# pandegroup/deepchem

Measured on AMD Instinct MI355X. Metric: molecules/sec fwd+bwd GraphConvModel, higher is better.
Workload: dtype f32; 1 GPU; Tox21-like synthetic molecules (18.2 atoms/mol, E/N 2.08), 12 binary tasks, GraphConvModel [64,64]/dense 128, BatchNorm on, fwd+bwd+Adam per step; grad_mode=full, gemm_mode=fast (split-bf16 x3 products on v_mfma_f32_32x32x16_bf16, fp32-accurate), parallelism=dp1 (molecules sharded by rank, one flat all-reduce per step)

## Files before the change

### deepchem_amd/_lib.py

```python
import ctypes
import os
from ctypes import (POINTER, Structure, c_char_p, c_double, c_float, c_int32, c_int64, c_void_p)

from deepchem_amd import _build

GCMI_MAX_DEG = 10
BN_ACC_REPLICAS = 32


def bn_acc_doubles(n_feat: int) -> int:
    return 66 * n_feat
K_GATHER_SUM, K_GATHER_MAX, K_READOUT, K_SEG_GEMM, K_WGRAD, K_GATHER_MAX_BWD, K_BATCHNORM, K_FUSED_BWD = 0, 1, 2, 3, 4, 5, 6, 7


GCMI_OPT_GEMM_EXACT = 1
GCMI_OPT_FUSED_BN_STATS = 2
GCMI_OPT_FUSED_BWD = 3
GCMI_OPT_FUSED_BWD_LAUNCHES = 4
GCMI_OPT_READOUT_PIPELINED = 5
GCMI_OPT_ONE_PIECE_LAUNCHES = 6
GCMI_OPT_MAX_SUM_LAUNCHES = 7
GCMI_METRIC_ROC_AUC, GCMI_METRIC_PRC_AUC = 0, 1
GCMI_METRIC_MOMENTS, GCMI_METRIC_ACCURACY = 0, 1
GCMI_METRIC_MOMENT_DOUBLES = 12
GCMI_WIN_META_INTS = 24
GCMI_COLLATE_WIN_DESC_INTS = 36
GCMI_WIN_MAX_SLOTS = 4095


class GcmiGraph(Structure):
    _fields_ = [
        ("n_atoms", c_int32),
        ("n_edges", c_int32),
        ("n_mols", c_int32),
        ("max_deg", c_int32),
        ("deg_start", c_int32 * (GCMI_MAX_DEG + 2)),
        ("edge_start", c_int32 * (GCMI_MAX_DEG + 2)),
        ("d_col_idx", c_void_p),
        ("d_membership", c_void_p),
        ("d_mol_runs", c_void_p),
        ("d_rev_pos", c_void_p),
        ("n_win", c_int32),
        ("n_win_big", c_int32),
        ("win_alloc", c_int32),
        ("win_ecap", c_int32),
        ("win_alloc_big", c_int32),
        ("win_ecap_big", c_int32),
        ("win_reserved", c_int32 * 2),
        ("d_win_meta", c_void_p),
        ("d_win_edges", c_void_p),
    ]


MAX_CONV_LAYERS = 4


class GcmiModelDesc(Structure):
    _fields_ = [
        ("n_layers", c_int32),
        ("max_deg", c_int32),
        ("n_feat_in", c_int32),
        ("conv_width", c_int32 * MAX_CONV_LAYERS),
        ("dense_width", c_int32),
        ("n_tasks", c_int32),
        ("n_classes", c_int32),
        ("mode", c_int32),
        ("batch_norm", c_int32),
        ("grad_mode", c_int32),
        ("bn_eps", c_float),
        ("bn_momentum", c_float),
        ("off_conv_w", c_int64 * MAX_CONV_LAYERS),
        ("off_conv_b", c_int64 * MAX_CONV_LAYERS),
        ("off_bn_gamma", c_int64 * (MAX_CONV_LAYERS + 1)),
        ("off_bn_beta", c_int64 * (MAX_CONV_LAYERS + 1)),
# ... 260 lines not shown
```

### deepchem_amd/csrc/bn.hip

```cpp
#include "common.h"
#include "split_bf16.h"

namespace gcmi {

constexpr int kBBlock = 256;
constexpr int kRowsPerBlock = 512;
constexpr int kResidentBlocks = 2048;
constexpr int kReplicas = kBnReplicas;

template <int V>
__device__ __forceinline__ void readout_dy(const ReadoutGrad& rg, int64_t r, int c, int n_feat, float (&dy)[V]) {
  const int m = rg.membership[r];
  const float* grow = rg.g2 + (int64_t)m * rg.ldg2;
  const int32_t* arow = rg.arg + (int64_t)m * n_feat;
  if constexpr (V == 4) {
    const float4 s4 = *reinterpret_cast<const float4*>(grow + c);
    const float4 m4 = *reinterpret_cast<const float4*>(grow + n_feat + c);
    const int4 a4 = *reinterpret_cast<const int4*>(arow + c);
    dy[0] = s4.x + (a4.x == r ? m4.x : 0.f);
    dy[1] = s4.y + (a4.y == r ? m4.y : 0.f);
    dy[2] = s4.z + (a4.z == r ? m4.z : 0.f);
    dy[3] = s4.w + (a4.w == r ? m4.w : 0.f);
  } else {
    dy[0] = grow[c] + (arow[c] == r ? grow[n_feat + c] : 0.f);
// ... 322 lines not shown
    const int c = cc * V;
    float A[V], B[V], C[V];
#pragma unroll
    for (int q = 0; q < V; ++q) {
      A[q] = coef[c + q];
      B[q] = coef[n_feat + c + q];
      C[q] = coef[2 * n_feat + c + q];
    }
    constexpr int R = 4;
    for (int64_t r0 = r_begin + ty; r0 < r_end; r0 += (int64_t)R * ry) {
      float xv[R][V], gv[R][V];
#pragma unroll
      for (int u = 0; u < R; ++u) {
        const int64_t r = r0 + (int64_t)u * ry;
        const int64_t rc = r < r_end ? r : r_end - 1;
        if constexpr (RD) readout_dy<V>(rg, rc, c, n_feat, gv[u]);
        if constexpr (V == 4) {
          const float4 a4 = *reinterpret_cast<const float4*>(x + rc * ldx + c);
          xv[u][0] = a4.x; xv[u][1] = a4.y; xv[u][2] = a4.z; xv[u][3] = a4.w;
          if (!RD) {
            const float4 b4 = *reinterpret_cast<const float4*>(dy + rc * lddy + c);
            gv[u][0] = b4.x; gv[u][1] = b4.y; gv[u][2] = b4.z; gv[u][3] = b4.w;
          }
        } else {
          xv[u][0] = x[rc * ldx + c];
          if (!RD) gv[u][0] = dy[rc * lddy + c];
        }
      }
#pragma unroll
      for (int u = 0; u < R; ++u) {
        const int64_t r = r0 + (int64_t)u * ry;
        if (r >= r_end) continue;
        float o[V];
#pragma unroll
        for (int q = 0; q < V; ++q) {
          const float v = fmaf(A[q], gv[u][q], fmaf(B[q], xv[u][q], C[q]));
          o[q] = (RELU && !(xv[u][q] > 0.f)) ? 0.f : v;
        }
        if constexpr (V == 4) {
          *reinterpret_cast<float4*>(dx + r * lddx + c) = make_float4(o[0], o[1], o[2], o[3]);
        } else {
          dx[r * lddx + c] = o[0];
        }
      }
    }
  }
}

static int launch_col_sums(int mode, const float* a, int64_t lda, const float* x, int64_t ldx,
                           const float* mean, const float* invstd, int64_t n_rows, int n_feat,
                           double* sums, bool acc_clean, hipStream_t st, const ReadoutGrad* rgp = nullptr,
                           const float* only_if_gamma = nullptr, const float* only_if_beta = nullptr, int x_bf16 = 0) {
  if (!acc_clean &&
      hipMemsetAsync(sums, 0, sizeof(double) * 2 * n_feat * (1 + kReplicas), st) != hipSuccess) {
    set_error("bn: memset failed");
    return GCMI_ERR_LAUNCH;
  }
  if (n_rows == 0) return GCMI_OK;
  ReadoutGrad rg{nullptr, nullptr, 0, nullptr};
  int V;
  if (rgp) {
    rg = *rgp;
    mode = 2;
    V = (vec_width(x, ldx, n_feat) == 4 && aligned16(rg.g2) && rg.ldg2 % 4 == 0 && aligned16(rg.arg)) ? 4 : 1;
  } else if (x_bf16) {
    const bool a_ok = x_bf16 == 2 ? ((reinterpret_cast<uintptr_t>(a) & 7u) == 0 && lda % 4 == 0 && n_feat % 4 == 0)
                                  : vec_width(a, lda, n_feat) == 4;
    if (mode != 1 || !a_ok || (reinterpret_cast<uintptr_t>(x) & 7u) || ldx % 4) {
      set_error("bn col_sums: bf16 rows need mode 1 and 8-byte addressable rows");
      return GCMI_ERR_UNSUPPORTED;
    }
    V = 4;
  } else {
    V = vec_width(a, lda, n_feat);
    if (mode == 1 && vec_width(x, ldx, n_feat) != 4) V = 1;
  }
  const int lpr = n_feat / V;
  const int lx = lpr < kBBlock ? lpr : kBBlock;
  const int64_t round_rows = 4 * (kBBlock / lx);
  int64_t rpb = (n_rows + kResidentBlocks - 1) / kResidentBlocks;
  if (rpb < kRowsPerBlock) rpb = kRowsPerBlock;
  rpb = (rpb + round_rows - 1) / round_rows * round_rows;
  const int blocks = (int)((n_rows + rpb - 1) / rpb);
  const int rev = next_sweep_direction();
#define LAUNCH_CS(VV, MM)                                                                     \
  hipLaunchKernelGGL((col_sums_kernel<VV, MM>), dim3(blocks), dim3(kBBlock), 0, st, a, lda, x, \
                     ldx, mean, invstd, n_rows, rpb, n_feat, lpr, lx, sums, rg, rev, only_if_gamma, only_if_beta)
  if (x_bf16 == 2) {
    hipLaunchKernelGGL((col_sums_kernel<4, 1, true, true>), dim3(blocks), dim3(kBBlock), 0, st, a, lda, x, ldx, mean, invstd,
                       n_rows, rpb, n_feat, lpr, lx, sums, rg, rev, only_if_gamma, only_if_beta);
  } else if (x_bf16) {
    hipLaunchKernelGGL((col_sums_kernel<4, 1, true>), dim3(blocks), dim3(kBBlock), 0, st, a, lda, x, ldx, mean, invstd,
                       n_rows, rpb, n_feat, lpr, lx, sums, rg, rev, only_if_gamma, only_if_beta);
  } else if (V == 4) {
    if (mode == 0) LAUNCH_CS(4, 0); else if (mode == 1) LAUNCH_CS(4, 1); else LAUNCH_CS(4, 2);
  } else {
    if (mode == 0) LAUNCH_CS(1, 0); else if (mode == 1) LAUNCH_CS(1, 1); else LAUNCH_CS(1, 2);
  }
#undef LAUNCH_CS
  GCMI_CHECK_LAUNCH("bn col_sums");
  return GCMI_OK;
}

static int bn_sync_collapse(const BnPoint& p, int64_t n_rows, double* d_acc, double* d_psums, double* d_xbuf, hipStream_t st,
                            const BnBackward::Loss& loss = {}) {
  static_assert(kReplicas == 32, "bn_collapse_kernel: one lane per replica");
  hipLaunchKernelGGL(bn_collapse_kernel, dim3((p.n_feat + 7) / 8), dim3(256), 0, st, d_acc, d_psums, n_rows, p.n_feat, p.gamma,
                     p.beta, p.dgamma, p.dbeta, d_xbuf, loss.acc, loss.rep, loss.inv_count, loss.out);
  GCMI_CHECK_LAUNCH("bn_collapse");
  return GCMI_OK;
}

static int bn_sync_exchange(const BnSync& sy, int64_t n_rows, int32_t n_feat, hipStream_t st) {
  const int64_t n = 2 * (int64_t)n_feat + 1;
  if (n_rows == 0 && hipMemsetAsync(sy.buf, 0, sizeof(double) * (size_t)n, st) != hipSuccess) {
    set_error("bn sync: memset failed");
    return GCMI_ERR_LAUNCH;
  }
  if (sy.fn(sy.ctx, sy.buf, n, st) != 0) {
    set_error("synchronised BatchNorm: the statistics exchange callback failed");
    return GCMI_ERR_LAUNCH;
  }
  return GCMI_OK;
}

static int bn_sync_finalize(const BnPoint& p, const double* d_xbuf, hipStream_t st) {
  hipLaunchKernelGGL(bn_finalize_sync_kernel, dim3((p.n_feat + 255) / 256), dim3(256), 0, st, d_xbuf, p.n_feat, p.gamma,
                     p.beta, p.eps, p.momentum, p.running_mean, p.running_var, p.mean, p.invstd, p.scale, p.shift,
                     p.batches_tracked);
  GCMI_CHECK_LAUNCH("bn_finalize_sync");
  return GCMI_OK;
}

int bn_train_forward(const BnPoint& p, const BnForward& f, void* stream) {
  const int32_t n_feat = p.n_feat;
  if (f.sync) {
    GCMI_CHECK_ARG(n_feat > 0 && f.n_rows >= 0 && p.scale && p.shift && f.acc && f.sync->fn && f.sync->buf,
                   "bn_stats_sync: bad arguments");
    GCMI_CHECK_ARG(f.n_rows == 0 || f.sums_ready || (f.x && f.ldx >= n_feat), "bn_stats_sync: bad rows");
  } else if (f.sums_ready) {
    GCMI_CHECK_ARG(n_feat > 0 && f.n_rows > 0 && p.scale && p.shift && f.acc, "bn_finalize: bad arguments");
  } else {
    GCMI_CHECK_ARG(n_feat > 0 && f.n_rows > 0 && f.ldx >= n_feat, "bn_stats: bad shape (n_rows=%lld)", (long long)f.n_rows);
    GCMI_CHECK_ARG(f.x && p.scale && p.shift && f.acc, "bn_stats: NULL buffer");
  }
  hipStream_t st = (hipStream_t)stream;
  TimedScope ts(GCMI_K_BATCHNORM, st);
  int rc = GCMI_OK;
  if (f.n_rows > 0 && !f.sums_ready)
    rc = launch_col_sums(0, f.x, f.ldx, nullptr, 0, nullptr, nullptr, f.n_rows, n_feat, f.acc, f.acc_clean, st);
  if (rc) return rc;
  if (!f.sync) {
    hipLaunchKernelGGL(bn_finalize_kernel, dim3((n_feat + 7) / 8), dim3(256), 0, st, f.acc, f.n_rows, n_feat, p.gamma, p.beta,
                       p.eps, p.momentum, p.running_mean, p.running_var, p.mean, p.invstd, p.scale, p.shift, p.batches_tracked);
    GCMI_CHECK_LAUNCH("bn_finalize");
    return GCMI_OK;
  }
  if (f.n_rows > 0) rc = bn_sync_collapse(BnPoint{n_feat}, f.n_rows, f.acc, nullptr, f.sync->buf, st);
  if (rc == GCMI_OK) rc = bn_sync_exchange(*f.sync, f.n_rows, n_feat, st);
  if (rc) return rc;
  return bn_sync_finalize(p, f.sync->buf, st);
}

static int bn_bwd_sync_finish(const BnPoint& p, const BnBackward& b, hipStream_t st) {
  const BnSync& sy = *b.sync;
  GCMI_CHECK_ARG(p.n_feat > 0 && b.n_rows > 0 && sy.fn && sy.buf, "bn_bwd_sync: bad arguments");
  GCMI_CHECK_ARG(p.mean && p.invstd && b.acc, "bn_bwd_sync: NULL buffer");
  int rc = bn_sync_collapse(p, b.n_rows, b.acc, b.psums, sy.buf, st, b.loss);
// ... 217 lines not shown
}

int bn_bwd_pool_impl(const BnPoint& p, const BnBackward& b, void* stream) {
  const int32_t n_feat = p.n_feat;
  GCMI_CHECK_ARG(n_feat > 0 && b.n_rows > 0 && p.mean && p.invstd && b.acc && b.psums && b.x && p.gamma && p.beta,
                 "bn_bwd_pool: bad arguments");
  hipStream_t st = (hipStream_t)stream;
  TimedScope ts(GCMI_K_BATCHNORM, st);
  if (b.dy != nullptr) {
    const int rc = launch_col_sums(1, b.dy, b.lddy, b.x, b.ldx, p.mean, p.invstd, b.n_rows, n_feat, b.acc, true, st, nullptr,
                                   p.gamma, p.beta, b.x_bf16);
    if (rc) return rc;
  }
  if (b.sync != nullptr) return bn_bwd_sync_finish(p, b, st);
  static_assert(kReplicas == 32, "bn_bwd_params_pool_kernel: one lane per replica");
  hipLaunchKernelGGL(bn_bwd_params_pool_kernel, dim3((n_feat + 7) / 8), dim3(256), 0, st, b.psums, b.acc, b.n_rows, n_feat,
                     p.gamma, p.beta, p.mean, p.invstd, p.dgamma, p.dbeta, reinterpret_cast<float*>(b.acc));
  GCMI_CHECK_LAUNCH("bn_bwd_params_pool");
  return GCMI_OK;
}

static int bn_bwd_params(const BnPoint& p, const BnBackward& b, hipStream_t st) {
  hipLaunchKernelGGL(bn_bwd_params_kernel, dim3((p.n_feat + 7) / 8), dim3(256), 0, st, b.acc, b.n_rows, p.n_feat, p.gamma,
                     p.mean, p.invstd, p.dgamma, p.dbeta, reinterpret_cast<float*>(b.acc), b.loss.acc, b.loss.rep,
                     b.loss.inv_count, b.loss.out);
  GCMI_CHECK_LAUNCH("bn_bwd_params");
  return GCMI_OK;
}

int bn_bwd_params_impl(const BnPoint& p, const BnBackward& b, void* stream) {
  GCMI_CHECK_ARG(p.n_feat > 0 && b.n_rows > 0 && p.mean && p.invstd && b.acc, "bn_bwd_params: bad arguments");
  hipStream_t st = (hipStream_t)stream;
  TimedScope ts(GCMI_K_BATCHNORM, st);
  return b.sync != nullptr ? bn_bwd_sync_finish(p, b, st) : bn_bwd_params(p, b, st);
}

int bn_bwd_impl(const BnPoint& p, const BnBackward& b, void* stream) {
  const int32_t n_feat = p.n_feat;
  const int64_t n_rows = b.n_rows;
  const ReadoutGrad* rgp = b.rg;
  if (rgp)
    GCMI_CHECK_ARG(rgp->membership && rgp->g2 && rgp->arg && rgp->ldg2 >= 2 * (int64_t)n_feat,
                   "bn_bwd_readout: bad readout gradient");
  else
    GCMI_CHECK_ARG(b.lddy >= n_feat && b.dy, "bn_bwd: bad dy");
  GCMI_CHECK_ARG(n_feat > 0 && n_rows > 0 && b.ldx >= n_feat, "bn_bwd: bad shape");
  GCMI_CHECK_ARG(b.x && p.mean && p.invstd && b.acc, "bn_bwd: NULL buffer");
  GCMI_CHECK_ARG(b.dx == nullptr || b.lddx >= n_feat, "bn_bwd: bad lddx");
  hipStream_t st = (hipStream_t)stream;
  TimedScope ts(GCMI_K_BATCHNORM, st);
  int rc = GCMI_OK;
  if (rgp && rgp->rawsum && rgp->runs && rgp->n_mols > 0) {
    if (!b.acc_clean &&
        hipMemsetAsync(b.acc, 0, sizeof(double) * 2 * n_feat * (1 + kReplicas), st) != hipSuccess) {
      set_error("bn: memset failed");
      return GCMI_ERR_LAUNCH;
    }
    const int chunks = (n_feat + 63) / 64;
    int waves = 4096 / chunks * chunks;
    const int64_t jobs = (int64_t)rgp->n_mols * chunks;
    if (jobs < waves) waves = (int)((jobs + chunks - 1) / chunks * chunks);
    const int blocks = (waves + 3) / 4;
    hipLaunchKernelGGL(readout_bn_sums_kernel, dim3(blocks), dim3(256), 0, st, rgp->n_mols, n_feat, rgp->n_deg,
                       rgp->runs, rgp->g2, rgp->ldg2, rgp->arg, rgp->rawsum, b.x, b.ldx, p.mean, p.invstd, chunks,
                       b.acc);
    GCMI_CHECK_LAUNCH("readout_bn_sums");
  } else {
    rc = launch_col_sums(1, b.dy, b.lddy, b.x, b.ldx, p.mean, p.invstd, n_rows, n_feat, b.acc, b.acc_clean, st, rgp);
  }
  if (rc) return rc;
  rc = b.sync != nullptr ? bn_bwd_sync_finish(p, b, st) : bn_bwd_params(p, b, st);
  if (rc) return rc;
  if (b.dx) {
    const float* coef = reinterpret_cast<const float*>(b.acc);
    ReadoutGrad rg{nullptr, nullptr, 0, nullptr};
    if (rgp) rg = *rgp;
    const bool src_ok = rgp ? (aligned16(rg.g2) && rg.ldg2 % 4 == 0 && aligned16(rg.arg))
                            : vec_width(b.dy, b.lddy, n_feat) == 4;
    const int V = (vec_width(b.dx, b.lddx, n_feat) == 4 && src_ok && vec_width(b.x, b.ldx, n_feat) == 4) ? 4 : 1;
    const int lpr = n_feat / V;
    const int lx = lpr < kBBlock ? lpr : kBBlock;
    const int64_t round_rows = 4 * (kBBlock / lx);
    int64_t rpb = (n_rows + kResidentBlocks - 1) / kResidentBlocks;
    if (rpb < kDxRows) rpb = kDxRows;
    rpb = (rpb + round_rows - 1) / round_rows * round_rows;
    const int blocks = (int)((n_rows + rpb - 1) / rpb);
    const int rev = next_sweep_direction();
#define LAUNCH_DX(VV, RR, DD)                                                                     \
  hipLaunchKernelGGL((bn_bwd_dx_kernel<VV, RR, DD>), dim3(blocks), dim3(kBBlock), 0, st, b.dy, b.lddy, \
                     b.x, b.ldx, n_rows, rpb, n_feat, lpr, lx, coef, b.dx, b.lddx, rg, rev)
#define LAUNCH_DX_R(VV, RR) \
  do { if (rgp) LAUNCH_DX(VV, RR, true); else LAUNCH_DX(VV, RR, false); } while (0)
    if (V == 4) {
      if (b.relu_mask) LAUNCH_DX_R(4, true); else LAUNCH_DX_R(4, false);
    } else {
      if (b.relu_mask) LAUNCH_DX_R(1, true); else LAUNCH_DX_R(1, false);
    }
#undef LAUNCH_DX_R
#undef LAUNCH_DX
    GCMI_CHECK_LAUNCH("bn_bwd_dx");
  }
  return GCMI_OK;
}

}
```

### deepchem_amd/csrc/bwd_fused.hip

```cpp
#include <atomic>
#include <type_traits>

#include "common.h"
#include "split_bf16.h"

namespace gcmi {

constexpr int kFRows = 64;

struct FusedArgs {
  const float* dy;
  int32_t lddy;
  const float* x;
  int32_t ldx;
  const float* coef;
  const int32_t* membership;
  const float* g2;
  int32_t ldg2;
  const int32_t* arg;
  const float* in[2];
  int32_t ldin[2];
  int32_t k_in;
  const float* w;
  float* dw;
// ... 519 lines not shown
    if (stamp) { t0 = wall_clock64(); d_w2 += t0 - t1; }
    prow0 = row0; pvalid = valid; pseg = seg;
    seg = nseg; row0 = nrow0; valid = nvalid;
    nseg = n2seg; nrow0 = n2row0; nvalid = n2valid;
  }
  store_out(prow0, pvalid, pseg);
  if (!is_dgrad) flush_w(cur_seg);
  if constexpr (DGRAD) {
    if (a.psums != nullptr) {
      flush_psums();
      __syncthreads();
      for (int c = tid; c < 2 * KP; c += NT) {
        const int which = c / KP, col = c - which * KP;
        if (col < a.k_in)
          atomicAdd(a.psums + (size_t)2 * a.k_in * (1 + (blockIdx.x % kBnReplicas)) + (size_t)which * a.k_in + col,
                    stat_s[which][col]);
      }
    }
  }
  if (stamp) {
    unsigned long long* d = a.diag + (wave == 0 ? 0 : 5);
    d[0] = d_a; d[1] = d_w1; d[2] = d_b; d[3] = d_w2; d[4] = (unsigned long long)my_tiles;
  }
}

static bool fused_bwd_on() {
  static const int env = getenv("GCMI_FUSED_BWD") ? atoi(getenv("GCMI_FUSED_BWD")) : 1;
  return env != 0;
}

static std::atomic<int> g_fused_bwd{1};
static std::atomic<int> g_fused_launches{0};
int fused_bwd_launches() { return g_fused_launches.load(std::memory_order_relaxed); }
void set_fused_bwd(int on) { g_fused_bwd.store(on ? 1 : 0, std::memory_order_relaxed); }
int get_fused_bwd() { return g_fused_bwd.load(std::memory_order_relaxed); }
bool fused_bwd_enabled() { return fused_bwd_on() && get_fused_bwd() != 0 && !gemm_exact_mode(); }

template <int NG, int KT, int NOPS, bool TRANS, bool RD, bool DGRAD, bool HB = false, bool GB = false, bool IB = HB>
static int launch_fused(const SegTable& st, int n_tiles, const FusedArgs& a, hipStream_t sm) {
  constexpr int KP = KT * 32;
  size_t shmem = sizeof(float) * kFRows * (NG + 4) + sizeof(float) * (size_t)NOPS * kFRows * (KP + 4);
  if (DGRAD)
    shmem += sizeof(unsigned short) * (size_t)NOPS * 3 * KP * (NG + 8) + sizeof(float) * kFRows * (NOPS * KT * 32 + 8);
  auto kern = fused_bwd_kernel<NG, KT, NOPS, TRANS, RD, DGRAD, HB, GB, IB>;
  static LdsLimit lim;
  if (!raise_lds_limit(lim, reinterpret_cast<const void*>(kern), shmem)) return GCMI_ERR_UNSUPPORTED;
  const int per_cu = DGRAD ? 1 : 2;
  const int grid = std::min(n_tiles, 256 * per_cu);
  static const bool diag_on = getenv("GCMI_FUSED_DIAG") && atoi(getenv("GCMI_FUSED_DIAG")) != 0;
  static unsigned long long* d_diag = nullptr;
  FusedArgs aa = a;
  if (diag_on) {
    if (!d_diag && hipMalloc(&d_diag, 10 * sizeof(unsigned long long)) != hipSuccess) d_diag = nullptr;
    if (d_diag) (void)hipMemsetAsync(d_diag, 0, 10 * sizeof(unsigned long long), sm);
    aa.diag = d_diag;
  }
  hipLaunchKernelGGL(kern, dim3(grid), dim3(DGRAD ? 512 : 256), shmem, sm, st, n_tiles, aa, next_sweep_direction());
  GCMI_CHECK_LAUNCH("fused_bwd");
  if (diag_on && d_diag) {
    unsigned long long h[10];
    if (hipStreamSynchronize(sm) == hipSuccess && hipMemcpy(h, d_diag, sizeof(h), hipMemcpyDeviceToHost) == hipSuccess)
      fprintf(stderr, "fused_bwd<%d,%d,%d> tiles %llu | first wave: G phase %.2f us, wait %.2f, products %.2f, wait %.2f "
                      "| last wave: %.2f %.2f %.2f %.2f (per tile)\n", NG, KT, (int)DGRAD, h[4],
              h[0] * 0.01 / h[4], h[1] * 0.01 / h[4], h[2] * 0.01 / h[4], h[3] * 0.01 / h[4], h[5] * 0.01 / h[4],
              h[6] * 0.01 / h[4], h[7] * 0.01 / h[4], h[8] * 0.01 / h[4]);
  }
  g_fused_launches.fetch_add(1, std::memory_order_relaxed);
  return GCMI_OK;
}

static FusedArgs fused_args(const BlockBackward& b) {
  FusedArgs a;
  memset(&a, 0, sizeof(a));
  a.dy = b.dy; a.lddy = (int32_t)b.lddy; a.x = b.gc; a.ldx = (int32_t)b.ldgc; a.coef = b.coef;
  if (b.rg) { a.membership = b.rg->membership; a.g2 = b.rg->g2; a.ldg2 = (int32_t)b.rg->ldg2; a.arg = b.rg->arg; }
  for (int o = 0; o < 2; ++o) {
    a.in[o] = b.in[o].rows; a.ldin[o] = (int32_t)b.in[o].ld;
    a.dout[o] = b.dout[o].rows; a.lddout[o] = (int32_t)b.dout[o].ld;
  }
  a.k_in = b.k_in; a.w = b.w; a.dw = b.dw; a.db = b.db;
  a.psums = b.dout[0].rows ? b.psums : nullptr;
  return a;
}

int fused_conv_bwd(const BlockBackward& b, hipStream_t sm) {
  const int32_t k_in = b.k_in, act_bf16 = b.act_bf16, in_bf16 = b.in_bf16;
  if (!fused_bwd_enabled() || b.n_seg > kMaxProductSeg || b.width != 64 || b.rg != nullptr) return GCMI_ERR_UNSUPPORTED;
  if (in_bf16 && (act_bf16 || b.dout[0].rows != nullptr || k_in <= 64 || k_in > 96)) return GCMI_ERR_UNSUPPORTED;
  {
    int64_t rows = 0;
    for (int sgi = 0; sgi < b.n_seg; ++sgi) rows = std::max<int64_t>(rows, b.seg_end[sgi]);
    const int64_t ldmax = std::max(std::max(b.lddy, b.ldgc),
                                   std::max(std::max(b.in[0].ld, b.in[1].ld), std::max(b.dout[0].ld, b.dout[1].ld)));
    if (rows * ldmax >= (int64_t)1 << 30) return GCMI_ERR_UNSUPPORTED;
  }
  if (!aligned16(b.dy) || b.lddy % 4 || !aligned16(b.gc) || b.ldgc % 4) return GCMI_ERR_UNSUPPORTED;
  if (b.coef && !aligned16(b.coef)) return GCMI_ERR_UNSUPPORTED;
  if ((act_bf16 || in_bf16) && (!aligned16(b.in[0].rows) || b.in[0].ld % 4 || !aligned16(b.in[1].rows) || b.in[1].ld % 4))
    return GCMI_ERR_UNSUPPORTED;
  const bool dgrad = b.dout[0].rows != nullptr;
  SegTable st;
  const int tiles = (int)fill_seg_table(st, b.n_seg, b.seg_begin, b.seg_end, b.w_off[0], b.w_off[1], b.b_off, kFRows);
  if (tiles == 0) return GCMI_OK;
  const FusedArgs a = fused_args(b);
  if (dgrad) {
    if (k_in % 4 || b.dout[0].ld % 4 || b.dout[1].ld % 4 || !aligned16(b.dout[0].rows) || !aligned16(b.dout[1].rows))
      return GCMI_ERR_UNSUPPORTED;
// ... 124 lines not shown
```

### deepchem_amd/csrc/collate.cpp

```cpp
#include <cmath>
#include <algorithm>
#include <cstdlib>
#include <string>
#include <thread>
#include <vector>

#include "common.h"

namespace {

constexpr int ND = GCMI_MAX_DEG + 1;

template <typename F>
void parallel_for(int64_t n, int n_threads, F&& fn) {
  if (n_threads <= 1 || n < 512) {
    fn(0, n, 0);
    return;
  }
  std::vector<std::thread> th;
  for (int t = 0; t < n_threads; ++t) th.emplace_back(fn, n * t / n_threads, n * (t + 1) / n_threads, t);
  for (auto& x : th) x.join();
}


// ... 686 lines not shown
    for (int d = 0; d < ND; ++d) {
      D[d] = W.begin[d];
      D[ND + d] = W.sb[d];
      D[2 * ND + d] = W.eb[d];
    }
    GCMI_CHECK_ARG(W.eoff < (1LL << 31), "collate: window entries exceed int32");
    D[3 * ND] = (int32_t)W.eoff;
    D[3 * ND + 1] = D[3 * ND + 2] = 0;
  }
  out_offsets[0] = o_base;
  out_offsets[1] = o_win;
  out_offsets[2] = o_off;
  out_offsets[3] = o_a0;
  out_offsets[4] = o_meta;
  out_offsets[5] = o_desc;
  out_offsets[6] = o_desc + n_win * WD;
  out_offsets[7] = P.want_win ? P.win_entries : 0;
  graph->n_atoms = (int32_t)P.n_atoms;
  graph->n_edges = (int32_t)P.n_edges;
  graph->n_mols = (int32_t)n_sel;
  graph->max_deg = max_deg;
  for (int d = 0; d < GCMI_MAX_DEG + 2; ++d) {
    graph->deg_start[d] = (int32_t)P.deg_start[d <= n_deg ? d : n_deg];
    graph->edge_start[d] = (int32_t)P.edge_start[d <= n_deg ? d : n_deg];
  }
  graph->d_col_idx = nullptr;
  graph->d_membership = nullptr;
  graph->d_mol_runs = nullptr;
  graph->d_rev_pos = nullptr;
  graph->n_win = (int32_t)n_win;
  graph->n_win_big = P.want_win ? P.n_win_big : 0;
  graph->win_alloc = P.want_win ? P.win_alloc : 0;
  graph->win_ecap = P.want_win ? P.win_ecap : 0;
  graph->win_alloc_big = P.want_win ? P.win_alloc_big : 0;
  graph->win_ecap_big = P.want_win ? P.win_ecap_big : 0;
  graph->win_reserved[0] = P.want_win ? P.n_mols_with_atoms : 0;
  graph->win_reserved[1] = 0;
  graph->d_win_meta = nullptr;
  graph->d_win_edges = nullptr;
  return GCMI_OK;
}

int gcmi_collate_rows(const void* d_features, int64_t n_feat, const int64_t* d_adj_ptr, const int32_t* d_adj_idx,
                      const int32_t* d_rank, const uint8_t* d_rev, const int32_t* d_staging, const int64_t* offsets,
                      const gcmi_graph* plan, float* d_out_features, int64_t out_ld, int32_t* d_membership,
                      int32_t* d_col_idx, int32_t* d_mol_runs, uint8_t* d_rev_pos, uint16_t* d_win_edges,
                      int64_t* d_src_atom, void* stream_) {
  hipStream_t stream = (hipStream_t)stream_;
  RowsArgs A;
  const int rc = fill_rows_args(A, d_features, n_feat, d_adj_ptr, d_adj_idx, d_rank, d_rev, d_staging, offsets, plan,
                                d_out_features, out_ld, d_membership, d_col_idx, d_mol_runs, d_rev_pos, d_win_edges);
  if (rc != GCMI_OK) return rc;
  if (A.want_win && offsets[7] > 0)
    if (hipMemsetAsync(d_win_edges, 0, (size_t)offsets[7] * sizeof(uint16_t), stream) != hipSuccess) {
      ::gcmi::set_error("collate_rows: hipMemsetAsync failed");
      return GCMI_ERR_LAUNCH;
    }
  A.src_atom = d_src_atom;
  if (A.n_atoms > 0) {
    collate_rows_kernel<<<(unsigned)((A.n_atoms + 255) / 256), 256, 0, stream>>>(A);
    GCMI_CHECK_LAUNCH("collate_rows_kernel");
    if (d_src_atom) {
      const int64_t n_el = (int64_t)A.n_atoms * A.out_ld;
      GCMI_CHECK_ARG(n_el / 256 < (1LL << 31), "collate_rows: feature block too large for one launch");
      if (A.out_ld % 4 == 0 && ((uintptr_t)A.out_feat & 15) == 0 && n_el / 4 < (1LL << 31)) {
        const uint32_t n_quads = (uint32_t)(n_el / 4);
        collate_features_quad_kernel<<<(n_quads + 255u) / 256u, 256, 0, stream>>>(A, (uint32_t)(A.out_ld / 4), n_quads);
      } else {
        collate_features_kernel<<<(unsigned)((n_el + 255) / 256), 256, 0, stream>>>(A);
      }
      GCMI_CHECK_LAUNCH("collate_features_kernel");
    }
  }
  const int64_t n_runs = (int64_t)A.n_sel * A.n_deg;
  if (d_mol_runs && n_runs > 0) {
    collate_runs_kernel<<<(unsigned)((n_runs + 255) / 256), 256, 0, stream>>>(A);
    GCMI_CHECK_LAUNCH("collate_runs_kernel");
  }
  return GCMI_OK;
}

int gcmi_collate_rows_host(const void* features, int64_t n_feat, const int64_t* adj_ptr, const int32_t* adj_idx,
                           const int32_t* rank, const uint8_t* rev, const int32_t* staging, const int64_t* offsets,
                           const gcmi_graph* plan, float* out_features, int64_t out_ld, int32_t* membership,
                           int32_t* col_idx, int32_t* mol_runs, uint8_t* rev_pos, uint16_t* win_edges) {
  RowsArgs A;
  const int rc = fill_rows_args(A, features, n_feat, adj_ptr, adj_idx, rank, rev, staging, offsets, plan, out_features,
                                out_ld, membership, col_idx, mol_runs, rev_pos, win_edges);
  if (rc != GCMI_OK) return rc;
  if (A.want_win)
    for (int64_t q = 0; q < offsets[7]; ++q) win_edges[q] = 0;
  for (int32_t i = 0; i < A.n_atoms; ++i) collate_atom(A, i);
  if (mol_runs)
    for (int64_t k = 0; k < (int64_t)A.n_sel * A.n_deg; ++k) collate_run(A, (int32_t)k);
  return GCMI_OK;
}

}

namespace {
inline int64_t up4w(int64_t n) { return (n + 3) / 4 * 4; }
}

extern "C" {

int64_t gcmi_collate_batches_layout(const int64_t* atom_ptr, const int64_t* adj_ptr, const int64_t* sel,
                                    const int64_t* batch_ptr, int64_t n_batches, int64_t ld, int32_t max_deg,
// ... 127 lines not shown
```

### deepchem_amd/csrc/common.h

```cpp
#pragma once
#include <hip/hip_runtime.h>
#include <algorithm>
#include <atomic>
#include <stdlib.h>
#include <stdint.h>
#include <stdio.h>
#include <string.h>

#include "../../include/gcmi.h"

namespace gcmi {

void set_error(const char* fmt, ...);
int next_sweep_direction();

constexpr int kMaxDev = 64;
struct LdsLimit {
  std::atomic<int> per_cu[kMaxDev];
};
int raise_lds_limit(LdsLimit& a, const void* kern, size_t lds_bytes, int threads = 0, size_t shmem = 0);

#define GCMI_CHECK_ARG(cond, ...)          \
  do {                                     \
    if (!(cond)) {                         \
      ::gcmi::set_error(__VA_ARGS__);      \
      return GCMI_ERR_ARG;                 \
    }                                      \
  } while (0)

#define GCMI_CHECK_LAUNCH(what)                                                        \
  do {                                                                                 \
    hipError_t e__ = hipGetLastError();                                                \
    if (e__ != hipSuccess) {                                                           \
      ::gcmi::set_error("%s: %s", what, hipGetErrorString(e__));                       \
      return GCMI_ERR_LAUNCH;                                                          \
    }                                                                                  \
  } while (0)

void timing_begin(int kernel_id, hipStream_t s);
void timing_end(int kernel_id, hipStream_t s);

struct TimedScope {
  int id;
  hipStream_t s;
  TimedScope(int id_, hipStream_t s_) : id(id_), s(s_) { timing_begin(id, s); }
  ~TimedScope() { timing_end(id, s); }
};

struct DegTable {
  int32_t max_deg;
  int32_t deg_start[GCMI_MAX_DEG + 2];
  int32_t edge_start[GCMI_MAX_DEG + 2];
};

inline DegTable make_deg_table(const gcmi_graph* g) {
  DegTable t;
  t.max_deg = g->max_deg;
  for (int d = 0; d < GCMI_MAX_DEG + 2; ++d) {
    t.deg_start[d] = g->deg_start[d < g->max_deg + 1 ? d : g->max_deg + 1];
    t.edge_start[d] = g->edge_start[d < g->max_deg + 1 ? d : g->max_deg + 1];
  }
  return t;
}

int check_graph(const gcmi_graph* g, bool need_cols);

bool win_usable(const gcmi_graph* g, int n_feat, bool aux);
bool win_has_width(int n_feat);
int win_gather_sum(const gcmi_graph* g, const float* d_x, int64_t ldx, int n_feat, float* d_s,
                   int64_t lds, hipStream_t st, bool accumulate = false);
int win_gather_max(const gcmi_graph* g, const float* d_x, int64_t ldx, int n_feat, const float* d_scale,
                   const float* d_shift, float* d_out, int64_t ldo, uint8_t* d_arg, hipStream_t st);
int win_gather_max_bwd(const gcmi_graph* g, const float* d_dout, int64_t lddo, int n_feat,
                       const uint8_t* d_arg, float* d_dx, int64_t lddx, hipStream_t st);
bool win_two_stage_usable(const gcmi_graph* g, int n_feat);
int win_gather_sumacc_max_bwd(const gcmi_graph* g, const float* d_ds, int64_t ldds, int n_feat, float* d_dxs,
                              int64_t lddxs, const uint8_t* d_arg, float* d_dy, int64_t lddy, hipStream_t st);
bool win_max_sum_usable(const gcmi_graph* g, int n_feat);
int win_gather_max_sum(const gcmi_graph* g, const float* d_y, int64_t ldy, int n_feat, const float* d_scale,
                       const float* d_shift, float* d_pool, int64_t ldp, uint8_t* d_arg, float* d_s, int64_t lds,
                       hipStream_t st);
int max_sum_launches();
int win_gather_max_bwd_if_ill(const gcmi_graph* g, const float* d_dout, int64_t lddo, int n_feat, const uint8_t* d_arg,
                              float* d_dx, int64_t lddx, const float* d_gamma, const float* d_beta, hipStream_t st);
// ... 413 lines not shown
```

### deepchem_amd/csrc/core.cpp

```cpp
#include <atomic>
#include <cstdlib>
#include <stdarg.h>

#include <mutex>
#include <vector>

#include "common.h"

namespace gcmi {

static thread_local char g_err[512] = "";

static std::atomic<unsigned> g_sweep_counter{0};
int next_sweep_direction() { return (int)(g_sweep_counter.fetch_add(1, std::memory_order_relaxed) & 1u); }

int raise_lds_limit(LdsLimit& a, const void* kern, size_t lds_bytes, int threads, size_t shmem) {
  int dev = -1;
  const bool keyed = hipGetDevice(&dev) == hipSuccess && dev >= 0 && dev < kMaxDev;
  if (keyed) {
    const int done = a.per_cu[dev].load(std::memory_order_relaxed);
    if (done > 0) return done;
  } else {
    (void)hipGetLastError();
  }
  if (hipFuncSetAttribute(kern, hipFuncAttributeMaxDynamicSharedMemorySize, (int)lds_bytes) != hipSuccess) {
    (void)hipGetLastError();
    return 0;
  }
  int per_cu = 1;
  if (threads > 0 && (hipOccupancyMaxActiveBlocksPerMultiprocessor(&per_cu, kern, threads, shmem) != hipSuccess ||
                      per_cu < 1)) {
    (void)hipGetLastError();
    per_cu = 2;
  }
  if (keyed) a.per_cu[dev].store(per_cu, std::memory_order_relaxed);
  return per_cu;
}

void set_error(const char* fmt, ...) {
  va_list ap;
  va_start(ap, fmt);
  vsnprintf(g_err, sizeof(g_err), fmt, ap);
  va_end(ap);
}

int check_graph(const gcmi_graph* g, bool need_cols) {
  GCMI_CHECK_ARG(g != nullptr, "graph is NULL");
  GCMI_CHECK_ARG(g->max_deg >= 0 && g->max_deg <= GCMI_MAX_DEG, "max_deg %d outside [0,%d]",
                 g->max_deg, GCMI_MAX_DEG);
  GCMI_CHECK_ARG(g->n_atoms >= 0 && g->n_edges >= 0 && g->n_mols >= 0, "negative graph size");
  GCMI_CHECK_ARG(g->deg_start[0] == 0 && g->edge_start[0] == 0, "deg_start/edge_start must begin at 0");
  int64_t e = 0;
  for (int d = 0; d <= g->max_deg; ++d) {
    int64_t nd = (int64_t)g->deg_start[d + 1] - g->deg_start[d];
    GCMI_CHECK_ARG(nd >= 0, "deg_start not ascending at degree %d", d);
    GCMI_CHECK_ARG(g->edge_start[d] == e, "edge_start[%d]=%d, expected %lld", d, g->edge_start[d],
                   (long long)e);
    e += nd * d;
  }
  GCMI_CHECK_ARG(g->deg_start[g->max_deg + 1] == g->n_atoms, "deg_start[max_deg+1]=%d != n_atoms=%d",
                 g->deg_start[g->max_deg + 1], g->n_atoms);
  GCMI_CHECK_ARG(e == g->n_edges && g->edge_start[g->max_deg + 1] == g->n_edges,
                 "n_edges=%d inconsistent with the degree blocks (%lld)", g->n_edges, (long long)e);
  if (need_cols) GCMI_CHECK_ARG(g->n_edges == 0 || g->d_col_idx != nullptr, "d_col_idx is NULL");
  return GCMI_OK;
}

// ... 67 lines not shown
```

### deepchem_amd/csrc/gather.hip

```cpp
#include "common.h"

namespace gcmi {

constexpr int kBlock = 256;
constexpr int kUnroll = 4;

struct TileTable {
  int32_t tile_start[GCMI_MAX_DEG + 2];
};

static int make_tiles(const gcmi_graph* g, int lpr, bool skip_deg0, TileTable* tt) {
  int64_t tiles = 0;
  const int64_t per_tile = (int64_t)kBlock * kUnroll;
  for (int d = 0; d <= GCMI_MAX_DEG + 1; ++d) {
    tt->tile_start[d] = (int32_t)tiles;
    if (d <= g->max_deg && !(skip_deg0 && d == 0)) {
      int64_t slots = (int64_t)(g->deg_start[d + 1] - g->deg_start[d]) * lpr;
      tiles += (slots + per_tile - 1) / per_tile;
    }
  }
  return (int)tiles;
}

__device__ __forceinline__ int block_degree(const TileTable& tt, int b) {
// ... 371 lines not shown
                    ? 4
                    : 1;
  if (V == 4 && win_has_width(n_feat) && win_usable(g, n_feat, false) &&
      (d_scale == nullptr || (aligned16(d_scale) && aligned16(d_shift)))) {
    TimedScope ts(GCMI_K_GATHER_MAX, st);
    return win_gather_max(g, d_x, ldx, n_feat, d_scale, d_shift, d_out, ldo, d_arg, st);
  }
  const int lpr = n_feat / V;
  TileTable tt;
  const int tiles = make_tiles(g, lpr, false, &tt);
  DegTable t = make_deg_table(g);
  const bool bn = d_scale != nullptr;
  TimedScope ts(GCMI_K_GATHER_MAX, st);
#define LAUNCH_GM(VV, BB)                                                                       \
  hipLaunchKernelGGL((gather_max_kernel<VV, BB>), dim3(tiles), dim3(kBlock), 0, st, t, tt,      \
                     g->d_col_idx, d_x, ldx, lpr, n_feat, d_scale, d_shift, d_out, ldo, d_arg)
  if (V == 4) {
    if (bn) LAUNCH_GM(4, true); else LAUNCH_GM(4, false);
  } else {
    if (bn) LAUNCH_GM(1, true); else LAUNCH_GM(1, false);
  }
#undef LAUNCH_GM
  GCMI_CHECK_LAUNCH("gather_max_fwd");
  return GCMI_OK;
}

int gcmi_gather_max_sum_fwd(const gcmi_graph* g, const float* d_y, int64_t ldy, int32_t n_feat,
                            const float* d_scale, const float* d_shift, float* d_pool, int64_t ldp,
                            uint8_t* d_arg, float* d_s, int64_t lds, void* stream) {
  int rc = check_graph(g, true);
  if (rc) return rc;
  GCMI_CHECK_ARG(n_feat > 0 && ldy >= n_feat && ldp >= n_feat && lds >= n_feat, "gather_max_sum: bad n_feat/ld");
  GCMI_CHECK_ARG(g->n_atoms == 0 || (d_y && d_pool && d_s), "gather_max_sum: NULL buffer");
  GCMI_CHECK_ARG((d_scale == nullptr) == (d_shift == nullptr), "gather_max_sum: scale/shift must come together");
  if (g->n_atoms == 0) return GCMI_OK;
  hipStream_t st = (hipStream_t)stream;
  const bool v4 = vec_width(d_y, ldy, n_feat) == 4 && vec_width(d_pool, ldp, n_feat) == 4 &&
                  vec_width(d_s, lds, n_feat) == 4 && (d_arg == nullptr || (reinterpret_cast<uintptr_t>(d_arg) & 3u) == 0) &&
                  (d_scale == nullptr || (aligned16(d_scale) && aligned16(d_shift)));
  if (v4 && win_max_sum_usable(g, n_feat)) {
    TimedScope ts(GCMI_K_GATHER_SUM, st);
    return win_gather_max_sum(g, d_y, ldy, n_feat, d_scale, d_shift, d_pool, ldp, d_arg, d_s, lds, st);
  }
  rc = gcmi_gather_max_fwd(g, d_y, ldy, n_feat, d_scale, d_shift, d_pool, ldp, d_arg, stream);
  if (rc) return rc;
  return gcmi_gather_sum_fwd(g, d_pool, ldp, n_feat, d_s, lds, 0, stream);
}

int gcmi_build_rev_pos(const gcmi_graph* g, uint8_t* d_rev_pos, int32_t* d_flag, void* stream) {
  int rc = check_graph(g, true);
  if (rc) return rc;
  GCMI_CHECK_ARG(d_flag != nullptr, "build_rev_pos: d_flag is NULL");
  hipStream_t st = (hipStream_t)stream;
  if (hipMemsetAsync(d_flag, 0, sizeof(int32_t), st) != hipSuccess) {
    set_error("build_rev_pos: memset failed");
    return GCMI_ERR_LAUNCH;
  }
  if (g->n_edges == 0) return GCMI_OK;
  GCMI_CHECK_ARG(d_rev_pos != nullptr, "build_rev_pos: NULL output");
  DegTable t = make_deg_table(g);
  hipLaunchKernelGGL(rev_pos_kernel, dim3(grid_for(g->n_edges, kBlock)), dim3(kBlock), 0, st, t,
                     g->n_edges, g->d_col_idx, d_rev_pos, d_flag);
  GCMI_CHECK_LAUNCH("build_rev_pos");
  return GCMI_OK;
}

int gcmi_gather_max_bwd(const gcmi_graph* g, const float* d_dout, int64_t lddo, int32_t n_feat,
                        const uint8_t* d_arg, float* d_dx, int64_t lddx, void* stream) {
  int rc = check_graph(g, true);
  if (rc) return rc;
  GCMI_CHECK_ARG(n_feat > 0 && lddo >= n_feat && lddx >= n_feat, "gather_max_bwd: bad n_feat/ld");
  GCMI_CHECK_ARG(g->n_atoms == 0 || (d_dout && d_arg && d_dx), "gather_max_bwd: NULL buffer");
  if (g->n_atoms == 0) return GCMI_OK;
  hipStream_t st = (hipStream_t)stream;
  const int V = (n_feat % 4 == 0 && vec_width(d_dout, lddo, n_feat) == 4 &&
                 vec_width(d_dx, lddx, n_feat) == 4 && (reinterpret_cast<uintptr_t>(d_arg) & 3u) == 0)
                    ? 4
                    : 1;
  const int lpr = n_feat / V;
  TileTable tt;
  const int tiles = make_tiles(g, lpr, false, &tt);
  DegTable t = make_deg_table(g);
  if (V == 4 && (g->d_rev_pos != nullptr || g->n_edges == 0) && win_has_width(n_feat) &&
      win_usable(g, n_feat, true)) {
    TimedScope ts(GCMI_K_GATHER_MAX_BWD, st);
    return win_gather_max_bwd(g, d_dout, lddo, n_feat, d_arg, d_dx, lddx, st);
  }
  if (g->d_rev_pos != nullptr || g->n_edges == 0) {
    TimedScope ts(GCMI_K_GATHER_MAX_BWD, st);
    if (V == 4)
      hipLaunchKernelGGL(gather_max_bwd_gather_kernel<4>, dim3(tiles), dim3(kBlock), 0, st, t, tt,
                         g->d_col_idx, g->d_rev_pos, d_dout, lddo, lpr, n_feat, d_arg, d_dx, lddx);
    else
      hipLaunchKernelGGL(gather_max_bwd_gather_kernel<1>, dim3(tiles), dim3(kBlock), 0, st, t, tt,
                         g->d_col_idx, g->d_rev_pos, d_dout, lddo, lpr, n_feat, d_arg, d_dx, lddx);
    GCMI_CHECK_LAUNCH("gather_max_bwd (gather form)");
    return GCMI_OK;
  }
  if (V == 4)
    hipLaunchKernelGGL(gather_max_bwd_kernel<4>, dim3(tiles), dim3(kBlock), 0, st, t, tt,
                       g->d_col_idx, d_dout, lddo, lpr, n_feat, d_arg, d_dx, lddx);
  else
    hipLaunchKernelGGL(gather_max_bwd_kernel<1>, dim3(tiles), dim3(kBlock), 0, st, t, tt,
                       g->d_col_idx, d_dout, lddo, lpr, n_feat, d_arg, d_dx, lddx);
  GCMI_CHECK_LAUNCH("gather_max_bwd");
  return GCMI_OK;
}
// ... 116 lines not shown
```

### deepchem_amd/csrc/gather_lds.hip

```cpp
#include "common.h"
#include "split_bf16.h"

namespace gcmi {

constexpr int kND = GCMI_MAX_DEG + 1;
constexpr int kLdsPerCU = 160 * 1024;
constexpr int kRingBytes = 320;
constexpr int kHeadBytes = kRingBytes + 2048;

typedef __attribute__((address_space(3))) void* lds_ptr_t;

__device__ __forceinline__ unsigned lds_addr(const void* p) {
  return __builtin_amdgcn_readfirstlane((unsigned)(size_t)(lds_ptr_t)p);
}
__device__ __forceinline__ void glds16(const void* gsrc, unsigned lds_dst) {
  unsigned keep;
  lds_dst = __builtin_amdgcn_readfirstlane(lds_dst);
  asm volatile("s_mov_b32 %0, m0\n\ts_mov_b32 m0, %2\n\ts_nop 0\n\tglobal_load_lds_dwordx4 %1, off\n\ts_mov_b32 m0, %0"
               : "=&s"(keep) : "v"(gsrc), "s"(lds_dst) : "memory");
}
__device__ __forceinline__ void glds4(const void* gsrc, unsigned lds_dst) {
  unsigned keep;
  lds_dst = __builtin_amdgcn_readfirstlane(lds_dst);
  asm volatile("s_mov_b32 %0, m0\n\ts_mov_b32 m0, %2\n\ts_nop 0\n\tglobal_load_lds_dword %1, off\n\ts_mov_b32 m0, %0"
// ... 382 lines not shown

template <bool BN>
struct MaxOp : MaxBody<float, BN> {
  static constexpr int kThreads = 256;
};
template <bool BN>
struct MaxOpH : MaxBody<bf16_t, BN> {
  static constexpr int kThreads = 512;
};

template <class Op, class T>
struct MaxBwdBody {
  using P = Piece<T>;
  T* __restrict__ dx;
  int64_t lddx;
  const float* __restrict__ only_if_gamma;
  const float* __restrict__ only_if_beta;
  static constexpr Third kThird = Third::none;
  __device__ __forceinline__ bool skip(int n_feat) const {
    return only_if_gamma != nullptr && !bn_pool_ill_conditioned(only_if_gamma, only_if_beta, n_feat);
  }
  template <int WT>
  __device__ __forceinline__ void init(float*, int) const {}
  template <int WT, int LPR>
  __device__ __forceinline__ void run(const char* buf, const Layout& L, const WinMeta& m, const float*) const {
    constexpr int kPre = Op::kPre;
    const WinBuf<P> w = open_buf<P, LPR>(buf, L, m);
    for (int e0 = threadIdx.x; e0 < w.n16; e0 += kPre * WT) {
#pragma unroll
      for (int k = 0; k < kPre; ++k) {
        const int e = e0 + k * WT;
        if (e >= w.n16) break;
        const PieceAt at = piece_at<LPR>(m, L.maxd, e);
        typename P::Vals acc;
        pool_bwd<P, LPR>(w.tile, w.aux, w.ent + at.eloc, at.d, e, at.c, acc);
        store_piece(dx + (int64_t)at.row * lddx + at.c * P::kEPP, acc);
      }
    }
  }
};

struct MaxBwdOp : MaxBwdBody<MaxBwdOp, float> {
  static constexpr int kThreads = 512;
  static constexpr int kPre = 4;
};
struct MaxBwdOpH : MaxBwdBody<MaxBwdOpH, bf16_t> {
  static constexpr int kThreads = 256;
  static constexpr int kPre = 1;
};

template <class T>
struct SumAccMaxBwdBody {
  using P = Piece<T>;
  const T* __restrict__ dxs;
  int64_t lddxs;
  T* __restrict__ dy;
  int64_t lddy;
  static constexpr Third kThird = Third::dma_pair;
  __device__ __forceinline__ const char* extra_src() const { return reinterpret_cast<const char*>(dxs); }
  __device__ __forceinline__ int64_t extra_ld_bytes() const { return lddxs * (int64_t)sizeof(T); }
  __device__ __forceinline__ bool skip(int) const { return false; }
  template <int WT>
  __device__ __forceinline__ void init(float*, int) const {}
  template <int WT, int LPR>
  __device__ __forceinline__ void run(const char* buf, const Layout& L, const WinMeta& m, char* extra) const {
    const WinBuf<P> w = open_buf<P, LPR>(buf, L, m);
    typename P::Raw* t2 = reinterpret_cast<typename P::Raw*>(extra);
    for (int e = threadIdx.x; e < w.n16; e += WT) {
      const PieceAt at = piece_at<LPR>(m, L.maxd, e);
      typename P::Vals acc;
      neigh_sum<P, LPR>(w.tile, w.ent + at.eloc, at.d, at.c, acc);
      add_piece<P>(acc, t2[e]);
      t2[e] = P::narrow(acc);
    }
    __syncthreads();
    for (int e = threadIdx.x; e < w.n16; e += WT) {
      const PieceAt at = piece_at<LPR>(m, L.maxd, e);
      typename P::Vals acc;
      pool_bwd<P, LPR>(t2, w.aux, w.ent + at.eloc, at.d, e, at.c, acc);
      store_piece(dy + (int64_t)at.row * lddy + at.c * P::kEPP, acc);
    }
  }
};

struct SumAccMaxBwdOp : SumAccMaxBwdBody<float> {
  static constexpr int kThreads = 1024;
};
struct SumAccMaxBwdOpH : SumAccMaxBwdBody<bf16_t> {
  static constexpr int kThreads = 512;
};

template <class T, bool BN>
struct MaxSumBody {
  using P = Piece<T>;
  MaxBody<T, BN> pool;
  T* __restrict__ s;
  int64_t lds;
  static constexpr Third kThird = Third::scratch;
  __device__ __forceinline__ bool skip(int) const { return false; }
  template <int WT>
  __device__ __forceinline__ void init(float* sh_lds, int n_feat) const { pool.template init<WT>(sh_lds, n_feat); }
  template <int WT, int LPR>
  __device__ __forceinline__ void run(const char* buf, const Layout& L, const WinMeta& m, const float* sh_lds,
                                      char* extra) const {
    const WinBuf<P> w = open_buf<P, LPR>(buf, L, m);
    typename P::Raw* t2 = reinterpret_cast<typename P::Raw*>(extra);
    for (int e = threadIdx.x; e < w.n16; e += WT) {
      const PieceAt at = piece_at<LPR>(m, L.maxd, e);
      typename P::Vals best;
      typename P::Bytes ba;
      pool_max<P, LPR, BN>(w.tile, w.ent + at.eloc, at.d, e, at.c, sh_lds, best, ba);
      store_piece(pool.out + (int64_t)at.row * pool.ldo + at.c * P::kEPP, best);
      if (pool.arg) P::store_arg(pool.arg + (int64_t)at.row * (LPR * P::kEPP) + at.c * P::kEPP, ba);
      t2[e] = P::narrow(best);
    }
    __syncthreads();
    for (int e = threadIdx.x; e < w.n16; e += WT) {
      const PieceAt at = piece_at<LPR>(m, L.maxd, e);
      typename P::Vals acc;
      neigh_sum<P, LPR>(t2, w.ent + at.eloc, at.d, at.c, acc);
      store_piece(s + (int64_t)at.row * lds + at.c * P::kEPP, acc);
    }
  }
};

template <bool BN, int WT>
struct MaxSumOp : MaxSumBody<float, BN> {
  static constexpr int kThreads = WT;
};

template <int WT, int LPR, bool AUX, class Op>
__global__ void __launch_bounds__(WT)
win_kernel(const int32_t* __restrict__ meta, const uint16_t* __restrict__ edges, int n_norm, int n_win,
           int g_norm, Layout L, Layout Lbig, const char* __restrict__ x, int64_t ldx,
           const uint8_t* __restrict__ aux, Op op, int rev) {
  extern __shared__ __attribute__((aligned(16))) char smem_all[];
  int(*ring)[GCMI_WIN_META_INTS] = reinterpret_cast<int(*)[GCMI_WIN_META_INTS]>(smem_all);
  float* op_lds = reinterpret_cast<float*>(smem_all + kRingBytes);
  char* smem = smem_all + kHeadBytes;
  constexpr int kEPP = Op::P::kEPP;
  constexpr bool kXT = Op::kThird == Third::dma_pair;
  constexpr bool kScratch = Op::kThird == Third::scratch;
  if (op.skip(LPR * kEPP)) return;
  op.template init<WT>(op_lds, LPR * kEPP);
  auto compute = [&](const char* buf, const Layout& l, const WinMeta& m, char* extra) {
    if constexpr (kXT) op.template run<WT, LPR>(buf, l, m, extra);
    else if constexpr (kScratch) op.template run<WT, LPR>(buf, l, m, op_lds, extra);
    else op.template run<WT, LPR>(buf, l, m, op_lds);
  };
  const int t = threadIdx.x;
  if ((int)blockIdx.x >= g_norm) {
    const int G = gridDim.x - g_norm;
    for (int w = n_norm + (int)blockIdx.x - g_norm; w < n_win; w += G) {
      if (t < GCMI_WIN_META_INTS) ring[0][t] = meta[(size_t)w * GCMI_WIN_META_INTS + t];
      __syncthreads();
      const WinMeta m = read_meta(ring[0]);
      stage<WT, LPR, AUX, kEPP>(smem, Lbig, m, x, ldx, aux, edges);
      wait_dma();
      __syncthreads();
      compute(smem, Lbig, m, smem + 2 * L.buf_bytes());
      __syncthreads();
    }
    return;
  }
  const int G = g_norm;
  int w = blockIdx.x;
  auto widx = [&](int v) { return (size_t)(rev ? n_norm - 1 - v : v); };
  const int bb = L.buf_bytes();
  int metareg = 0;
  if (t < GCMI_WIN_META_INTS) {
    ring[0][t] = meta[widx(w) * GCMI_WIN_META_INTS + t];
    if (w + G < n_norm) ring[1][t] = meta[widx(w + G) * GCMI_WIN_META_INTS + t];
    if (w + 2 * G < n_norm) metareg = meta[widx(w + 2 * G) * GCMI_WIN_META_INTS + t];
  }
  __syncthreads();
  stage<WT, LPR, AUX, kEPP>(smem, L, read_meta(ring[0]), x, ldx, aux, edges);
  if constexpr (kXT) stage_extra<WT, LPR>(smem + 2 * bb, L, read_meta(ring[0]), op.extra_src(), op.extra_ld_bytes());
  int it = 0;
  for (;;) {
    wait_dma();
    __syncthreads();
    const bool has_next = w + G < n_norm;
    if (t < GCMI_WIN_META_INTS) {
      ring[(it + 2) % 3][t] = metareg;
      if (w + 3 * G < n_norm) metareg = meta[widx(w + 3 * G) * GCMI_WIN_META_INTS + t];
    }
    if (has_next) {
      stage<WT, LPR, AUX, kEPP>(smem + ((it + 1) & 1) * bb, L, read_meta(ring[(it + 1) % 3]), x, ldx, aux, edges);
      if constexpr (kXT)
        stage_extra<WT, LPR>(smem + 2 * bb + ((it + 1) & 1) * L.tile_bytes, L, read_meta(ring[(it + 1) % 3]), op.extra_src(),
                             op.extra_ld_bytes());
    }
    compute(smem + (it & 1) * bb, L, read_meta(ring[it % 3]), smem + 2 * bb + (kXT ? (it & 1) * L.tile_bytes : 0));
    if (!has_next) break;
    w += G;
    ++it;
  }
}

static bool windows_disabled() {
  static int v = -1;
  if (v < 0) v = getenv("GCMI_NO_WINDOWS") != nullptr ? 1 : 0;
  return v == 1;
}

static Layout make_layout(int alloc, int ecap, int maxd, int n_feat, int aux) {
  Layout L;
  L.tile_bytes = alloc * n_feat * 4;
  L.aux_bytes = aux == 4 ? (alloc * n_feat + 15) / 16 * 16 : aux == 8 ? (alloc * (n_feat / 4) + 63) / 64 * 512 : 0;
  L.edge_bytes = (ecap > 8 ? ecap : 8) * 2;
  L.maxd = maxd;
  return L;
}

struct WinPlan {
  Layout L, Lbig;
  size_t shmem;
  bool ok;
};

static WinPlan make_plan(const gcmi_graph* g, int n_feat, int aux) {
  int maxd = 0;
  for (int d = 1; d <= g->max_deg; ++d)
    if (g->deg_start[d + 1] > g->deg_start[d]) maxd = d;
  WinPlan p;
  p.Lbig = make_layout(g->win_alloc_big, g->win_ecap_big, maxd, n_feat, aux);
  int alloc = std::max(g->win_alloc, 1);
  p.L = make_layout(alloc, g->win_ecap, maxd, n_feat, aux);
  if (g->n_win_big > 0) {
    while (2 * p.L.buf_bytes() < p.Lbig.buf_bytes()) {
      alloc += 8;
      p.L = make_layout(alloc, g->win_ecap, maxd, n_feat, aux);
    }
  }
  p.shmem = 2 * (size_t)p.L.buf_bytes() + kHeadBytes;
  p.ok = p.shmem <= (size_t)kLdsPerCU;
  return p;
}

static bool plan_fits(const gcmi_graph* g, int n_floats, int aux) {
  if (windows_disabled() || g->d_win_meta == nullptr || g->n_win <= 0) return false;
  if (g->d_win_edges == nullptr || g->n_win_big < 0 || g->n_win_big > g->n_win) return false;
  return make_plan(g, n_floats, aux).ok;
}
static bool third_tiles_fit(const gcmi_graph* g, int n_floats, int aux, Third kind) {
  const WinPlan p = make_plan(g, n_floats, aux);
  return p.shmem + (size_t)third_tiles(kind) * p.L.tile_bytes <= (size_t)kLdsPerCU;
}

template <int LPR, bool AUX, class Op>
static int launch_lpr(const gcmi_graph* g, const WinPlan& p, const char* x, int64_t ldx, const uint8_t* aux,
                      const Op& op, hipStream_t st, const char* what, int which) {
  constexpr int WT = Op::kThreads;
  auto kern = win_kernel<WT, LPR, AUX, Op>;
  static LdsLimit lim;
  if (!raise_lds_limit(lim, reinterpret_cast<const void*>(kern), kLdsPerCU)) {
    set_error("%s: cannot raise the dynamic LDS limit", what);
    return GCMI_ERR_LAUNCH;
  }
  const int n_norm = g->n_win - g->n_win_big;
  size_t shmem = p.shmem;
  if constexpr (Op::kThird != Third::none) {
    if (which != 1) {
      set_error("%s: oversized windows are not handled by the two-stage form", what);
      return GCMI_ERR_UNSUPPORTED;
    }
    shmem += (size_t)p.L.tile_bytes * third_tiles(Op::kThird);
    if (shmem > (size_t)kLdsPerCU) return GCMI_ERR_UNSUPPORTED;
  }
  const int by_lds = (int)((size_t)kLdsPerCU / shmem);
  const int by_threads = 2048 / WT;
  const int per_cu = std::max(1, std::min(8, std::min(by_lds, by_threads)));
  const int g_norm = which == 2 ? 0 : std::min(n_norm, 256 * per_cu);
  const int g_big = which == 1 ? 0 : std::min(g->n_win_big, 64);
  if (g_norm + g_big == 0) return GCMI_OK;
  const int rev = next_sweep_direction();
  if constexpr (Op::kThird == Third::scratch) (void)next_sweep_direction();
  hipLaunchKernelGGL(kern, dim3(g_norm + g_big), dim3(WT), shmem, st, g->d_win_meta, g->d_win_edges, n_norm,
                     g->n_win, g_norm, p.L, p.Lbig, x, ldx, aux, op, rev);
  GCMI_CHECK_LAUNCH(what);
  return GCMI_OK;
}

template <bool AUX, class T, class Op>
static int launch(const gcmi_graph* g, int n_feat, const T* x, int64_t ldx, const uint8_t* aux, const Op& op,
                  hipStream_t st, const char* what, int which = 0) {
  using P = Piece<T>;
  constexpr bool kH = P::kEPP == 8;
  const WinPlan p = make_plan(g, n_feat * (int)sizeof(T) / 4, AUX ? P::kEPP : 0);
  const char* xb = reinterpret_cast<const char*>(x);
  const int64_t ldb = ldx * (int64_t)sizeof(T);
  switch (n_feat / P::kEPP) {
    case 8: if constexpr (kH) return launch_lpr<8, AUX, Op>(g, p, xb, ldb, aux, op, st, what, which); break;
    case 10: if constexpr (kH) return launch_lpr<10, AUX, Op>(g, p, xb, ldb, aux, op, st, what, which); break;
    case 16: return launch_lpr<16, AUX, Op>(g, p, xb, ldb, aux, op, st, what, which);
    case 19: if constexpr (!kH) return launch_lpr<19, AUX, Op>(g, p, xb, ldb, aux, op, st, what, which); break;
    case 32: if constexpr (!kH) return launch_lpr<32, AUX, Op>(g, p, xb, ldb, aux, op, st, what, which); break;
    default: break;
  }
  set_error(kH ? "%s: no bf16 window kernel for %d features" : "%s: no window kernel for %d features", what, n_feat);
  return GCMI_ERR_UNSUPPORTED;
}

template <class TwoStage, class SumAcc, class Bwd, class T>
static int sumacc_max_bwd(const gcmi_graph* g, const T* d_ds, int64_t ldds, int n_feat, T* d_dxs, int64_t lddxs,
                          const uint8_t* d_arg, T* d_dy, int64_t lddy, hipStream_t st, const char* const (&what)[3]) {
  TwoStage op{{d_dxs, lddxs, d_dy, lddy}};
  int rc = launch<true>(g, n_feat, d_ds, ldds, d_arg, op, st, what[0], 1);
  if (rc || g->n_win_big == 0) return rc;
  SumAcc acc{{d_dxs, lddxs}};
  rc = launch<false>(g, n_feat, d_ds, ldds, nullptr, acc, st, what[1], 2);
  if (rc) return rc;
  Bwd mb{{d_dy, lddy, nullptr, nullptr}};
  return launch<true>(g, n_feat, d_dxs, lddxs, d_arg, mb, st, what[2], 2);
}

bool win_has_width(int n_feat) { return n_feat == 64 || n_feat == 76 || n_feat == 128; }

bool win_usable(const gcmi_graph* g, int n_feat, bool aux) {
  if (n_feat % 4 != 0 || n_feat > 256) return false;
  return plan_fits(g, n_feat, aux ? 4 : 0);
}

int win_gather_sum(const gcmi_graph* g, const float* d_x, int64_t ldx, int n_feat, float* d_s,
                   int64_t lds, hipStream_t st, bool accumulate) {
  if (accumulate) {
    SumOp<true> op{{d_s, lds}};
    return launch<false>(g, n_feat, d_x, ldx, nullptr, op, st, "win_gather_sum (accumulate)");
  }
  SumOp<false> op{{d_s, lds}};
  return launch<false>(g, n_feat, d_x, ldx, nullptr, op, st, "win_gather_sum");
}

int win_gather_max(const gcmi_graph* g, const float* d_x, int64_t ldx, int n_feat, const float* d_scale,
                   const float* d_shift, float* d_out, int64_t ldo, uint8_t* d_arg, hipStream_t st) {
  if (d_scale) {
    MaxOp<true> op{{d_scale, d_shift, d_out, ldo, d_arg}};
    return launch<false>(g, n_feat, d_x, ldx, nullptr, op, st, "win_gather_max");
  }
  MaxOp<false> op{{nullptr, nullptr, d_out, ldo, d_arg}};
  return launch<false>(g, n_feat, d_x, ldx, nullptr, op, st, "win_gather_max");
}

int win_gather_max_bwd(const gcmi_graph* g, const float* d_dout, int64_t lddo, int n_feat,
                       const uint8_t* d_arg, float* d_dx, int64_t lddx, hipStream_t st) {
  MaxBwdOp op{{d_dx, lddx, nullptr, nullptr}};
  return launch<true>(g, n_feat, d_dout, lddo, d_arg, op, st, "win_gather_max_bwd");
}

int win_gather_max_bwd_if_ill(const gcmi_graph* g, const float* d_dout, int64_t lddo, int n_feat, const uint8_t* d_arg,
                              float* d_dx, int64_t lddx, const float* d_gamma, const float* d_beta, hipStream_t st) {
  MaxBwdOp op{{d_dx, lddx, d_gamma, d_beta}};
  return launch<true>(g, n_feat, d_dout, lddo, d_arg, op, st, "win_gather_max_bwd (conditional)");
}

bool win_two_stage_usable(const gcmi_graph* g, int n_feat) {
  return win_has_width(n_feat) && win_usable(g, n_feat, true) && third_tiles_fit(g, n_feat, 4, Third::dma_pair);
}

int win_gather_sumacc_max_bwd(const gcmi_graph* g, const float* d_ds, int64_t ldds, int n_feat, float* d_dxs,
                              int64_t lddxs, const uint8_t* d_arg, float* d_dy, int64_t lddy, hipStream_t st) {
  return sumacc_max_bwd<SumAccMaxBwdOp, SumOp<true>, MaxBwdOp>(
      g, d_ds, ldds, n_feat, d_dxs, lddxs, d_arg, d_dy, lddy, st,
      {"win_gather_sumacc_max_bwd", "win_gather_sum (accumulate, oversized windows)",
       "win_gather_max_bwd (oversized windows)"});
}

bool win_max_sum_usable(const gcmi_graph* g, int n_feat) {
  return win_has_width(n_feat) && (n_feat == 64 || n_feat == 128) && win_usable(g, n_feat, false) &&
         third_tiles_fit(g, n_feat, 0, Third::scratch);
}

static std::atomic<int> g_max_sum_launches{0};
int max_sum_launches() { return g_max_sum_launches.load(std::memory_order_relaxed); }

template <bool BN>
static int max_sum(const gcmi_graph* g, const float* d_y, int64_t ldy, int n_feat, const MaxBody<float, BN>& pool,
                   float* d_s, int64_t lds, hipStream_t st) {
  const WinPlan p = make_plan(g, n_feat, 0);
  const char* yb = reinterpret_cast<const char*>(d_y);
  const int64_t ldb = ldy * (int64_t)sizeof(float);
  if (n_feat == 128) {
    MaxSumOp<BN, 1024> op{{pool, d_s, lds}};
    return launch_lpr<32, false>(g, p, yb, ldb, nullptr, op, st, "win_gather_max_sum", 1);
  }
  if (n_feat == 64) {
    MaxSumOp<BN, 512> op{{pool, d_s, lds}};
    return launch_lpr<16, false>(g, p, yb, ldb, nullptr, op, st, "win_gather_max_sum", 1);
  }
  set_error("win_gather_max_sum: no window kernel for %d features", n_feat);
  return GCMI_ERR_UNSUPPORTED;
}

int win_gather_max_sum(const gcmi_graph* g, const float* d_y, int64_t ldy, int n_feat, const float* d_scale,
                       const float* d_shift, float* d_pool, int64_t ldp, uint8_t* d_arg, float* d_s, int64_t lds,
                       hipStream_t st) {
  int rc = d_scale ? max_sum<true>(g, d_y, ldy, n_feat, {d_scale, d_shift, d_pool, ldp, d_arg}, d_s, lds, st)
                   : max_sum<false>(g, d_y, ldy, n_feat, {nullptr, nullptr, d_pool, ldp, d_arg}, d_s, lds, st);
  if (rc) return rc;
  if (g->n_win > g->n_win_big) g_max_sum_launches.fetch_add(1, std::memory_order_relaxed);
  if (g->n_win_big == 0) return rc;
  if (d_scale) {
    MaxOp<true> mx{{d_scale, d_shift, d_pool, ldp, d_arg}};
    rc = launch<false>(g, n_feat, d_y, ldy, nullptr, mx, st, "win_gather_max (oversized windows)", 2);
  } else {
    MaxOp<false> mx{{nullptr, nullptr, d_pool, ldp, d_arg}};
    rc = launch<false>(g, n_feat, d_y, ldy, nullptr, mx, st, "win_gather_max (oversized windows)", 2);
  }
  if (rc) return rc;
  SumOp<false> sm{{d_s, lds}};
  return launch<false>(g, n_feat, d_pool, ldp, nullptr, sm, st, "win_gather_sum (oversized windows)", 2);
}

bool win_usable_h(const gcmi_graph* g, int n_feat) {
  if (n_feat != 64 && n_feat != 80 && n_feat != 128) return false;
  return plan_fits(g, n_feat / 2, 0);
}

int win_gather_sum_fh(const gcmi_graph* g, const float* d_x, int64_t ldx, int n_feat, bf16_t* d_s, bf16_t* d_xcopy,
                      int64_t ldo, hipStream_t st) {
  if (n_feat % 4 != 0 || ldo < n_feat || (ldo - n_feat) % 4 != 0 || ldo % 8 != 0 || !aligned16(d_s) || !aligned16(d_xcopy)) {
    set_error("win_gather_sum (fp32 -> bf16): bad shape (n_feat %d, ldo %lld)", n_feat, (long long)ldo);
    return GCMI_ERR_UNSUPPORTED;
  }
  SumOpFH op{d_s, d_xcopy, ldo, (int)((ldo - n_feat) / 4)};
  return launch<false>(g, n_feat, d_x, ldx, nullptr, op, st, "win_gather_sum (fp32 -> bf16)");
}

int win_gather_sum_h(const gcmi_graph* g, const bf16_t* d_x, int64_t ldx, int n_feat, bf16_t* d_s, int64_t lds,
                     hipStream_t st, bool accumulate) {
  if (accumulate) {
    SumAccOpH op{{d_s, lds}};
    return launch<false>(g, n_feat, d_x, ldx, nullptr, op, st, "win_gather_sum (bf16, accumulate)");
  }
  SumOpH op{{d_s, lds}};
  return launch<false>(g, n_feat, d_x, ldx, nullptr, op, st, "win_gather_sum (bf16)");
}

int win_gather_max_h(const gcmi_graph* g, const bf16_t* d_x, int64_t ldx, int n_feat, const float* d_scale,
                     const float* d_shift, bf16_t* d_out, int64_t ldo, uint8_t* d_arg, hipStream_t st) {
  if (d_scale) {
    MaxOpH<true> op{{d_scale, d_shift, d_out, ldo, d_arg}};
    return launch<false>(g, n_feat, d_x, ldx, nullptr, op, st, "win_gather_max (bf16)");
  }
  MaxOpH<false> op{{nullptr, nullptr, d_out, ldo, d_arg}};
  return launch<false>(g, n_feat, d_x, ldx, nullptr, op, st, "win_gather_max (bf16)");
}

bool win_usable_gh(const gcmi_graph* g, int n_feat) { return n_feat == 64 && plan_fits(g, n_feat / 2, 8); }

int win_gather_max_bwd_h(const gcmi_graph* g, const bf16_t* d_dout, int64_t lddo, int n_feat, const uint8_t* d_arg,
                         bf16_t* d_dx, int64_t lddx, const float* only_if_gamma, const float* only_if_beta, hipStream_t st) {
  MaxBwdOpH op{{d_dx, lddx, only_if_gamma, only_if_beta}};
  return launch<true>(g, n_feat, d_dout, lddo, d_arg, op, st, "win_gather_max_bwd (bf16)");
}

bool win_two_stage_usable_h(const gcmi_graph* g, int n_feat) {
  return win_usable_gh(g, n_feat) && third_tiles_fit(g, n_feat / 2, 8, Third::dma_pair);
}

bool win_usable_bwd_h(const gcmi_graph* g, int n_feat) {
  if (n_feat != 64 && n_feat != 80 && n_feat != 128) return false;
  return plan_fits(g, n_feat / 2, 8);
}
bool win_two_stage_usable_bwd_h(const gcmi_graph* g, int n_feat) {
  return win_usable_bwd_h(g, n_feat) && third_tiles_fit(g, n_feat / 2, 8, Third::dma_pair);
}

int win_gather_sumacc_max_bwd_h(const gcmi_graph* g, const bf16_t* d_ds, int64_t ldds, int n_feat, bf16_t* d_dxs,
                                int64_t lddxs, const uint8_t* d_arg, bf16_t* d_dy, int64_t lddy, hipStream_t st) {
  return sumacc_max_bwd<SumAccMaxBwdOpH, SumAccOpH, MaxBwdOpH>(
      g, d_ds, ldds, n_feat, d_dxs, lddxs, d_arg, d_dy, lddy, st,
      {"win_gather_sumacc_max_bwd (bf16)", "win_gather_sum (bf16, accumulate, oversized windows)",
       "win_gather_max_bwd (bf16, oversized windows)"});
}

}
```

### deepchem_amd/csrc/gemm.hip

```cpp
#include <atomic>

#include "common.h"
#include "split_bf16.h"

namespace gcmi {

constexpr int kGBlock = 256;
constexpr int BM = 64;
constexpr int BNT = 64;
constexpr int KC = 32;
constexpr int BM2 = 128;

template <bool VEC4>
__device__ __forceinline__ void stage_a(float (*As)[KC + 1], const float* __restrict__ a,
                                        int64_t lda, int row0, int rows_valid, int k0, int K) {
  const int tid = threadIdx.x;
  if constexpr (VEC4) {
    const int kq = (tid & 7) * 4;
#pragma unroll
    for (int pass = 0; pass < 2; ++pass) {
      const int r = (tid >> 3) + pass * 32;
      float4 v = make_float4(0.f, 0.f, 0.f, 0.f);
      if (r < rows_valid && k0 + kq < K) {
        v = *reinterpret_cast<const float4*>(a + (int64_t)(row0 + r) * lda + k0 + kq);
// ... 491 lines not shown
#define LAUNCH_SG(TT, VV)                                                                        \
  hipLaunchKernelGGL((seg_gemm_kernel<TT, VV>), grid, dim3(kGBlock), 0, sm, st, a1.a, a1.ld, a1.k, \
                     a1.w, a2.a, a2.ld, a2.k, a2.w, p.bias, n_out, p.act, p.out, p.ldo)
    if (p.trans_w) LAUNCH_SG(true, false); else LAUNCH_SG(false, false);
#undef LAUNCH_SG
  }
  GCMI_CHECK_LAUNCH("seg_gemm");
  return GCMI_OK;
}

int seg_gemm_stats(const SegProduct<float>& p, double* d_stats, bool* fused, hipStream_t sm, float* d_wimg_scratch) {
  *fused = false;
  double* stats = g_fused_bn_stats.load(std::memory_order_relaxed) != 0 ? d_stats : nullptr;
  const bool fast = check_seg_product(p) == GCMI_OK && (p.act == 0 || p.act == 1) && !gemm_exact_mode();
  if (fast) {
    TimedScope ts(GCMI_K_SEG_GEMM, sm);
    const int rc = fwd_fused_gemm(p, stats, sm, d_wimg_scratch);
    if (rc != GCMI_ERR_UNSUPPORTED) {
      *fused = rc == GCMI_OK && stats != nullptr;
      return rc;
    }
  }
  if (fast && stats) {
    TimedScope ts(GCMI_K_SEG_GEMM, sm);
    const int rc = launch_seg_gemm4(p, sm, stats);
    if (rc != GCMI_ERR_UNSUPPORTED) {
      *fused = rc == GCMI_OK;
      return rc;
    }
  }
  return seg_gemm(p, sm);
}

}

using namespace gcmi;

extern "C" {

int gcmi_set_option(int32_t option, int32_t value) {
  GCMI_CHECK_ARG(option == GCMI_OPT_GEMM_EXACT || option == GCMI_OPT_FUSED_BN_STATS || option == GCMI_OPT_FUSED_BWD ||
                     option == GCMI_OPT_READOUT_PIPELINED,
                 "set_option: unknown option %d", option);
  if (option == GCMI_OPT_GEMM_EXACT) g_gemm_exact.store(value != 0 ? 1 : 0, std::memory_order_relaxed);
  else if (option == GCMI_OPT_FUSED_BN_STATS) g_fused_bn_stats.store(value != 0 ? 1 : 0, std::memory_order_relaxed);
  else if (option == GCMI_OPT_READOUT_PIPELINED) set_readout_pipelined(value);
  else set_fused_bwd(value);
  return GCMI_OK;
}

int gcmi_get_option(int32_t option, int32_t* value) {
  GCMI_CHECK_ARG((option == GCMI_OPT_GEMM_EXACT || option == GCMI_OPT_FUSED_BN_STATS || option == GCMI_OPT_FUSED_BWD ||
                  option == GCMI_OPT_FUSED_BWD_LAUNCHES || option == GCMI_OPT_READOUT_PIPELINED ||
                  option == GCMI_OPT_ONE_PIECE_LAUNCHES || option == GCMI_OPT_MAX_SUM_LAUNCHES) && value,
                 "get_option: unknown option %d", option);
  if (option == GCMI_OPT_GEMM_EXACT) *value = g_gemm_exact.load(std::memory_order_relaxed);
  else if (option == GCMI_OPT_FUSED_BN_STATS) *value = g_fused_bn_stats.load(std::memory_order_relaxed);
  else if (option == GCMI_OPT_FUSED_BWD) *value = get_fused_bwd();
  else if (option == GCMI_OPT_READOUT_PIPELINED) *value = get_readout_pipelined();
  else if (option == GCMI_OPT_ONE_PIECE_LAUNCHES) *value = one_piece_launches();
  else if (option == GCMI_OPT_MAX_SUM_LAUNCHES) *value = max_sum_launches();
  else *value = fused_bwd_launches();
  return GCMI_OK;
}

int gcmi_seg_gemm(int32_t n_seg, const int32_t* seg_begin, const int32_t* seg_end,
                  const float* d_a1, int64_t lda1, int32_t k1, const float* d_w1,
                  const int64_t* w1_off, const float* d_a2, int64_t lda2, int32_t k2,
                  const float* d_w2, const int64_t* w2_off, const float* d_bias,
                  const int64_t* bias_off, int32_t n_out, int32_t trans_w, int32_t act,
                  float* d_out, int64_t ldo, void* stream) {
  const SegProduct<float> p{n_seg, seg_begin, seg_end, {{d_a1, lda1, k1, d_w1, w1_off}, {d_a2, lda2, k2, d_w2, w2_off}},
                            d_bias, bias_off, n_out, trans_w, act, d_out, ldo};
  return seg_gemm(p, (hipStream_t)stream);
}

int64_t gcmi_fwd_fused_scratch_floats(void) { return kFwdHWimgFloats; }

int gcmi_fwd_fused_gemm(int32_t n_seg, const int32_t* seg_begin, const int32_t* seg_end,
                        const float* d_a1, int64_t lda1, int32_t k1, const float* d_w1,
                        const int64_t* w1_off, const float* d_a2, int64_t lda2, int32_t k2,
                        const float* d_w2, const int64_t* w2_off, const float* d_bias,
                        const int64_t* bias_off, int32_t n_out, int32_t trans_w, int32_t act,
                        float* d_out, int64_t ldo, double* d_stats, float* d_wimg_scratch, void* stream) {
  const SegProduct<float> p{n_seg, seg_begin, seg_end, {{d_a1, lda1, k1, d_w1, w1_off}, {d_a2, lda2, k2, d_w2, w2_off}},
                            d_bias, bias_off, n_out, trans_w, act, d_out, ldo};
  const int rc_args = check_seg_product(p);
  if (rc_args != GCMI_OK) return rc_args;
  GCMI_CHECK_ARG(d_wimg_scratch == nullptr || aligned16(d_wimg_scratch), "fwd_fused_gemm: the scratch must be 16-byte aligned");
  const int rc = fwd_fused_gemm(p, d_stats, (hipStream_t)stream, d_wimg_scratch);
  if (rc == GCMI_ERR_UNSUPPORTED)
    set_error("fwd_fused_gemm: exact mode, the one-pass kernels switched off, or a shape the persistent forward kernels "
              "do not cover (no other kernel stands behind this entry)");
  return rc;
}

int gcmi_fwd_fused_gemm_h(int32_t n_seg, const int32_t* seg_begin, const int32_t* seg_end,
                          const uint16_t* d_a1, int64_t lda1, int32_t k1, const float* d_w1,
                          const int64_t* w1_off, const uint16_t* d_a2, int64_t lda2, int32_t k2,
                          const float* d_w2, const int64_t* w2_off, const float* d_bias,
                          const int64_t* bias_off, int32_t n_out, int32_t trans_w, int32_t act,
                          void* d_out, int64_t ldo, int32_t out_f32, double* d_stats, float* d_wimg_scratch,
                          void* stream) {
  GCMI_CHECK_ARG(out_f32 == 0 || out_f32 == 1, "fwd_fused_gemm_h: out_f32 must be 0 (bf16 rows) or 1 (float rows)");
  GCMI_CHECK_ARG(d_wimg_scratch != nullptr && aligned16(d_wimg_scratch),
                 "fwd_fused_gemm_h: NULL or misaligned weight-image scratch");
  int rc;
  if (out_f32) {
    const SegProduct<uint16_t, float> p{n_seg, seg_begin, seg_end,
                                        {{d_a1, lda1, k1, d_w1, w1_off}, {d_a2, lda2, k2, d_w2, w2_off}},
                                        d_bias, bias_off, n_out, trans_w, act, static_cast<float*>(d_out), ldo};
    const int rc_args = check_seg_product(p);
    if (rc_args != GCMI_OK) return rc_args;
    rc = fwd_h_gemm(p, d_stats, d_wimg_scratch, (hipStream_t)stream);
// ... 166 lines not shown
```

### deepchem_amd/csrc/loss.hip

```cpp
#include <math.h>

#include <algorithm>

#include "common.h"

namespace gcmi {

constexpr int kLBlock = 256;

__device__ __forceinline__ double block_sum(double v, double* red) {
#pragma unroll
  for (int o = 32; o > 0; o >>= 1) v += __shfl_down(v, o);
  const int wave = threadIdx.x >> 6, lane = threadIdx.x & 63;
  if (lane == 0) red[wave] = v;
  __syncthreads();
  double t = 0.0;
  if (threadIdx.x == 0)
    for (int w = 0; w < kLBlock / 64; ++w) t += red[w];
  return t;
}

__global__ void __launch_bounds__(kLBlock)
loss_kernel(int kind, const float* __restrict__ logits, const float* __restrict__ labels,
            const float* __restrict__ weights, int64_t n_items, int n_classes, float inv_count,
// ... 33 lines not shown
  if (threadIdx.x == 0) atomicAdd(acc, t);
}

__global__ void loss_finalize_kernel(double* __restrict__ acc, float inv_count,
                                     float* __restrict__ loss, int n_rep) {
  if (threadIdx.x == 0 && blockIdx.x == 0) {
    double t = 0.0;
    for (int i = 0; i < n_rep; ++i) {
      t += acc[i];
      acc[i] = 0.0;
    }
    *loss = (float)(t * (double)inv_count);
  }
}

__global__ void __launch_bounds__(kLBlock)
softmax_kernel(const float* __restrict__ logits, int64_t n_items, int n_classes,
               float* __restrict__ probs) {
  for (int64_t it = (int64_t)blockIdx.x * kLBlock + threadIdx.x; it < n_items;
       it += (int64_t)gridDim.x * kLBlock) {
    const float* x = logits + it * n_classes;
    float m = -INFINITY;
    for (int c = 0; c < n_classes; ++c) m = fmaxf(m, x[c]);
    float se = 0.f;
    for (int c = 0; c < n_classes; ++c) se += expf(x[c] - m);
    const float inv = 1.f / se;
    for (int c = 0; c < n_classes; ++c) probs[it * n_classes + c] = expf(x[c] - m) * inv;
  }
}

__global__ void __launch_bounds__(kLBlock)
adam_kernel(float* __restrict__ p, const float* __restrict__ g, float* __restrict__ m,
            float* __restrict__ v, int64_t n, float one_minus_b1, float b2, float one_minus_b2,
            float step_size, float inv_bc2_sqrt, float eps) {
  for (int64_t i = (int64_t)blockIdx.x * kLBlock + threadIdx.x; i < n;
       i += (int64_t)gridDim.x * kLBlock) {
    const float gi = g[i];
    const float mi = m[i] + (gi - m[i]) * one_minus_b1;
    const float vi = v[i] * b2 + gi * gi * one_minus_b2;
    m[i] = mi;
    v[i] = vi;
    const float denom = sqrtf(vi) * inv_bc2_sqrt + eps;
    p[i] -= step_size * (mi / denom);
  }
}

int loss_impl(int32_t kind, const float* d_logits, const float* d_labels, const float* d_weights,
              int64_t n_rows, int32_t n_tasks, int32_t n_classes, float* d_loss, float* d_dlogits,
              float* d_probs, double* d_acc, bool acc_clean, void* stream) {
  GCMI_CHECK_ARG(kind == 0 || kind == 1, "loss: kind must be 0 (softmax CE) or 1 (L2)");
  GCMI_CHECK_ARG(n_rows > 0 && n_tasks > 0 && (kind == 1 || n_classes > 0), "loss: bad shape");
  GCMI_CHECK_ARG(d_logits && d_labels && d_loss && d_acc, "loss: NULL buffer");
  hipStream_t st = (hipStream_t)stream;
  if (!acc_clean && hipMemsetAsync(d_acc, 0, sizeof(double), st) != hipSuccess) {
    set_error("loss: memset failed");
    return GCMI_ERR_LAUNCH;
  }
  const int64_t n_items = n_rows * n_tasks;
  const float inv_count = 1.f / (float)n_items;
  const int loss_blocks = std::min(grid_for(n_items, kLBlock), 256);
  hipLaunchKernelGGL(loss_kernel, dim3(loss_blocks), dim3(kLBlock), 0, st, kind,
                     d_logits, d_labels, d_weights, n_items, kind == 0 ? n_classes : 1, inv_count,
                     d_dlogits, kind == 0 ? d_probs : nullptr, d_acc);
  GCMI_CHECK_LAUNCH("loss");
  hipLaunchKernelGGL(loss_finalize_kernel, dim3(1), dim3(64), 0, st, d_acc, inv_count, d_loss, 1);
  GCMI_CHECK_LAUNCH("loss_finalize");
  return GCMI_OK;
}

int loss_finalize_impl(double* d_acc, float inv_count, float* d_loss, void* stream, int n_rep) {
  hipLaunchKernelGGL(loss_finalize_kernel, dim3(1), dim3(64), 0, (hipStream_t)stream, d_acc, inv_count, d_loss, n_rep);
  GCMI_CHECK_LAUNCH("loss_finalize");
  return GCMI_OK;
}

}

using namespace gcmi;

extern "C" {

int gcmi_loss_fwd_bwd(int32_t kind, const float* d_logits, const float* d_labels,
                      const float* d_weights, int64_t n_rows, int32_t n_tasks,
                      int32_t n_classes, float* d_loss, float* d_dlogits, float* d_probs,
                      double* d_acc, void* stream) {
  return loss_impl(kind, d_logits, d_labels, d_weights, n_rows, n_tasks, n_classes, d_loss, d_dlogits,
                   d_probs, d_acc, false, stream);
}

int gcmi_softmax(const float* d_logits, int64_t n_rows_tasks, int32_t n_classes, float* d_probs,
                 void* stream) {
  GCMI_CHECK_ARG(n_rows_tasks >= 0 && n_classes > 0, "softmax: bad shape");
  if (n_rows_tasks == 0) return GCMI_OK;
  GCMI_CHECK_ARG(d_logits && d_probs, "softmax: NULL buffer");
  hipLaunchKernelGGL(softmax_kernel, dim3(grid_for(n_rows_tasks, kLBlock)), dim3(kLBlock), 0,
                     (hipStream_t)stream, d_logits, n_rows_tasks, n_classes, d_probs);
  GCMI_CHECK_LAUNCH("softmax");
  return GCMI_OK;
}

int gcmi_adam_step(float* d_param, const float* d_grad, float* d_m, float* d_v, int64_t n,
                   float lr, float beta1, float beta2, float eps, int64_t step, void* stream) {
  GCMI_CHECK_ARG(n >= 0 && step >= 1, "adam: bad n/step");
  if (n == 0) return GCMI_OK;
  GCMI_CHECK_ARG(d_param && d_grad && d_m && d_v, "adam: NULL buffer");
  const double bc1 = 1.0 - pow((double)beta1, (double)step);
  const double bc2 = 1.0 - pow((double)beta2, (double)step);
// ... 11 lines not shown
```

### deepchem_amd/csrc/metrics.hip

```cpp
#include <math.h>

#include "common.h"

namespace gcmi {

constexpr int kRadixBits = 8;
constexpr int kRadix = 1 << kRadixBits;
constexpr int kSortBlock = 256;
constexpr int kSortTile = 2048;
constexpr int kScanBlock = 1024;
constexpr int kScanWaves = kScanBlock / 64;

struct RankWorkspace {
  uint32_t* keys[2];
  uint32_t* rows[2];
  uint32_t* hist;
  int64_t tiles;
};

inline int64_t align16(int64_t b) { return (b + 15) & ~(int64_t)15; }

inline int64_t rank_tiles(int64_t n) { return (n + kSortTile - 1) / kSortTile; }

inline RankWorkspace carve(void* ws, int64_t n, int32_t n_tasks) {
// ... 286 lines not shown
        acc[6] += w * fabs(e);
        acc[7] += w * e * e;
      } else {
        int best = 0;
        float top = x[0];
        for (int c = 1; c < n_classes; ++c)
          if (x[c] > top) {
            top = x[c];
            best = c;
          }
        if ((double)best == y) acc[8] += w;
      }
    }
  }
  for (int k = 0; k < kMomSums; ++k) {
    __syncthreads();
    red[threadIdx.x] = acc[k];
    __syncthreads();
    if (ty == 0 && live_t) {
      double s = 0.0;
      for (int j = 0; j < rows_per_pass; ++j) s += red[j * lanes_t + tx];
      double* o = out + (int64_t)t * GCMI_METRIC_MOMENT_DOUBLES;
      atomicAdd(&o[k == 8 ? 10 : k], s);
      if (k == 0 && blockIdx.y == 0) {
        o[8] = y0;
        o[9] = p0;
      }
    }
  }
}

}

using namespace gcmi;

extern "C" {

int64_t gcmi_metrics_workspace_bytes(int64_t n, int32_t n_tasks) {
  if (n <= 0 || n_tasks <= 0) return 0;
  const int64_t seg = align16(n * n_tasks * (int64_t)sizeof(uint32_t));
  return 4 * seg + align16((int64_t)n_tasks * kRadix * rank_tiles(n) * (int64_t)sizeof(uint32_t));
}

int gcmi_metric_rank(int32_t which, const float* d_scores, int64_t row_stride, int64_t elem_stride,
                     const double* d_labels, int32_t positive, const float* d_weights, int64_t n, int32_t n_tasks,
                     double* d_out, int32_t* d_status, void* d_workspace, void* stream) {
  GCMI_CHECK_ARG(which == GCMI_METRIC_ROC_AUC || which == GCMI_METRIC_PRC_AUC, "metric_rank: which must be 0 (ROC) or 1 (PRC)");
  GCMI_CHECK_ARG(n > 0 && n < ((int64_t)1 << 31) && n_tasks > 0 && n_tasks <= 65535, "metric_rank: bad shape");
  GCMI_CHECK_ARG(row_stride >= 0 && elem_stride >= 0, "metric_rank: negative stride");
  GCMI_CHECK_ARG(d_scores && d_labels && d_out && d_status && d_workspace, "metric_rank: NULL buffer");
  GCMI_CHECK_ARG(aligned16(d_workspace), "metric_rank: workspace must be 16-byte aligned");
  hipStream_t st = (hipStream_t)stream;
  RankWorkspace ws = carve(d_workspace, n, n_tasks);
  if (hipMemsetAsync(d_status, 0, sizeof(int32_t) * n_tasks, st) != hipSuccess) {
    set_error("metric_rank: memset failed");
    return GCMI_ERR_LAUNCH;
  }
  const int64_t tiles = ws.tiles;
  GCMI_CHECK_ARG(tiles < ((int64_t)1 << 31), "metric_rank: too many rows");
  const int key_blocks = (int)std::min<int64_t>((n + kSortBlock - 1) / kSortBlock, 1024);
  hipLaunchKernelGGL(rank_keys_kernel, dim3(key_blocks, n_tasks), dim3(kSortBlock), 0, st, d_scores, row_stride,
                     elem_stride, n, n_tasks, ws.keys[0], ws.rows[0], d_status);
  GCMI_CHECK_LAUNCH("rank_keys");
  int cur = 0;
  for (int pass = 0; pass < 32 / kRadixBits; ++pass) {
    const int shift = pass * kRadixBits;
    hipLaunchKernelGGL(radix_hist_kernel, dim3((unsigned)tiles, n_tasks), dim3(kSortBlock), 0, st, ws.keys[cur], n, shift,
                       tiles, ws.hist);
    GCMI_CHECK_LAUNCH("radix_hist");
    hipLaunchKernelGGL(radix_offsets_kernel, dim3(n_tasks), dim3(kRadix), 0, st, ws.hist, tiles);
    GCMI_CHECK_LAUNCH("radix_offsets");
    hipLaunchKernelGGL(radix_scatter_kernel, dim3((unsigned)tiles, n_tasks), dim3(kSortBlock), 0, st, ws.keys[cur],
                       ws.rows[cur], n, shift, tiles, ws.hist, ws.keys[cur ^ 1], ws.rows[cur ^ 1]);
    GCMI_CHECK_LAUNCH("radix_scatter");
    cur ^= 1;
  }
  if (d_weights)
    hipLaunchKernelGGL((rank_scan_kernel<double, true>), dim3(n_tasks), dim3(kScanBlock), 0, st, which, ws.keys[cur],
                       ws.rows[cur], n, n_tasks, d_labels, (double)positive, d_weights, d_out, d_status);
  else
    hipLaunchKernelGGL((rank_scan_kernel<long long, false>), dim3(n_tasks), dim3(kScanBlock), 0, st, which, ws.keys[cur],
                       ws.rows[cur], n, n_tasks, d_labels, (double)positive, d_weights, d_out, d_status);
  GCMI_CHECK_LAUNCH("rank_scan");
  return GCMI_OK;
}

int gcmi_metric_moments(int32_t which, const float* d_pred, int64_t row_stride, int64_t elem_stride, int32_t n_classes,
                        const double* d_labels, const float* d_weights, const double* d_scale, const double* d_shift,
                        int64_t n, int32_t n_tasks, double* d_out, void* stream) {
  GCMI_CHECK_ARG(which == GCMI_METRIC_MOMENTS || which == GCMI_METRIC_ACCURACY,
                 "metric_moments: which must be 0 (moments) or 1 (accuracy)");
  GCMI_CHECK_ARG(n > 0 && n_tasks > 0, "metric_moments: bad shape");
  GCMI_CHECK_ARG(which == GCMI_METRIC_MOMENTS || n_classes >= 1, "metric_moments: accuracy needs n_classes >= 1");
  GCMI_CHECK_ARG(row_stride >= 0 && elem_stride >= 0, "metric_moments: negative stride");
  GCMI_CHECK_ARG(d_pred && d_labels && d_out, "metric_moments: NULL buffer");
  hipStream_t st = (hipStream_t)stream;
  if (hipMemsetAsync(d_out, 0, sizeof(double) * GCMI_METRIC_MOMENT_DOUBLES * n_tasks, st) != hipSuccess) {
    set_error("metric_moments: memset failed");
    return GCMI_ERR_LAUNCH;
  }
  int lanes_t = 1;
  while (lanes_t < n_tasks && lanes_t < 64) lanes_t <<= 1;
  const int rows_per_pass = kMomBlock / lanes_t;
  const int task_blocks = (n_tasks + lanes_t - 1) / lanes_t;
  const int row_blocks = (int)std::min<int64_t>((n + rows_per_pass - 1) / rows_per_pass, 64);
  hipLaunchKernelGGL(moments_kernel, dim3(task_blocks, row_blocks), dim3(kMomBlock), 0, st, which, d_pred, row_stride,
                     elem_stride, n_classes, d_labels, d_weights, d_scale, d_shift, n, n_tasks, lanes_t, d_out);
  GCMI_CHECK_LAUNCH("metric_moments");
  return GCMI_OK;
}

}
```

### deepchem_amd/csrc/model.hip

```cpp
#include <map>
#include <mutex>

#include "common.h"
#include "split_bf16.h"

namespace gcmi {

constexpr int kMaxL = GCMI_MAX_CONV_LAYERS;

struct BiasLayers {
  const float* src[kMaxL];
  float* dst[kMaxL];
  int width[kMaxL];
};

__global__ void bias_pack_kernel(BiasLayers bl, int max_deg) {
  const int l = blockIdx.y;
  const float* __restrict__ b_list = pick_n(bl.src, l);
  float* __restrict__ bsum = pick_n(bl.dst, l);
  const int width = pick_n(bl.width, l);
  if (b_list == nullptr) return;
  const int n = (max_deg + 1) * width;
  for (int i = blockIdx.x * blockDim.x + threadIdx.x; i < n; i += gridDim.x * blockDim.x) {
    const int d = i / width, c = i - d * width;
    bsum[i] = d == 0 ? b_list[(2 * max_deg) * width + c]
                     : b_list[(2 * (d - 1)) * width + c] + b_list[(2 * (d - 1) + 1) * width + c];
  }
}

__global__ void bias_unpack_kernel(BiasLayers bl, int max_deg) {
  const int l = blockIdx.y;
  const float* __restrict__ dbsum = pick_n(bl.src, l);
  float* __restrict__ db_list = pick_n(bl.dst, l);
  const int width = pick_n(bl.width, l);
  if (dbsum == nullptr) return;
  const int n = (2 * max_deg + 1) * width;
  for (int i = blockIdx.x * blockDim.x + threadIdx.x; i < n; i += gridDim.x * blockDim.x) {
    const int k = i / width, c = i - k * width;
    const int d = k == 2 * max_deg ? 0 : k / 2 + 1;
    db_list[i] = dbsum[d * width + c];
  }
}

__global__ void small_int_count_kernel(const float* __restrict__ x, int64_t ld, int64_t n_rows, int n_cols, float limit,
                                       unsigned long long* __restrict__ count) {
  const int64_t total = n_rows * n_cols;
  unsigned bad = 0;
  for (int64_t i = (int64_t)blockIdx.x * blockDim.x + threadIdx.x; i < total; i += (int64_t)gridDim.x * blockDim.x) {
    const int64_t r = i / n_cols;
    const float v = x[r * ld + (i - r * n_cols)];
    bad += (fabsf(v) <= limit && v == truncf(v)) ? 0u : 1u;
  }
  for (int o = 32; o > 0; o >>= 1) bad += __shfl_xor(bad, o);
  if ((threadIdx.x & 63) == 0 && bad) atomicAdd(count, (unsigned long long)bad);
}

struct CounterPtrs {
  int64_t* p[kMaxL + 1];
  int n;
};
__global__ void bump_counters_kernel(CounterPtrs c) {
  const int i = threadIdx.x;
  if (i < c.n && c.p[i] != nullptr) *c.p[i] += 1;
}

struct Ws {
  int64_t S[kMaxL], gc[kMaxL], pool[kMaxL], arg[kMaxL], bsum[kMaxL], bnv[kMaxL + 1];
  int64_t ldS[kMaxL], ngather[kMaxL];
  int64_t dense, arg_r, rsum, dfp, tA, tB, tC, tD, tE, total;
  int64_t xb;
  int64_t wimg;
  int64_t himg;
  int64_t dlogits, dbsum[kMaxL], lacc, acc, acc2, z_end;
  int64_t xch;
};

constexpr int64_t kOnePieceLd = 80;

static Ws carve(const gcmi_model_desc* m, int64_t N, int64_t B, int64_t ld_features) {
  Ws w;
// ... 121 lines not shown
  } while (0)


struct Block {
  int K, W;
  const float *w, *bias;
  float *dw, *dbias;
  float* dbias_rows;
  BnPoint bn;
};

struct Step {
  const gcmi_model_desc* m;
  const gcmi_graph* g;
  const gcmi_model_io* io;
  const float* d_params;
  float* d_grads;
  hipStream_t st;
  int L, storage;
  int64_t N, B;
  int32_t nN;
  Ws w;
  float* ws;
  Block blk[kMaxL + 1];
  double *acc, *acc2, *lacc;
  BnSync sync_s;
  const BnSync* sy;
  int32_t training;
  double* stats;
  const float *d_labels, *d_weights;
  int64_t n_rows;
  int64_t *grad_lo, *grad_hi;
  float loss_inv_count;
  bool full;
  bool sym;
  bool one_piece;
  ReadoutGrad rg;
  BiasLayers ub;

  Step() = default;
  Step(const Step&) = delete;
  bool bn() const { return m->batch_norm != 0; }
  bf16_t* H(int64_t off) const { return reinterpret_cast<bf16_t*>(ws + off); }
  const float* HF(int64_t off) const { return ws + off; }
  static bf16_t* HG(float* p) { return reinterpret_cast<bf16_t*>(p); }
  float* dpool() const { return ws + w.tC; }
  float* dX() const { return ws + w.tC; }
  float* dS() const { return ws + w.tE; }
  float* dy() const { return ws + w.tD; }
  float* dgc() const { return bn() ? ws + w.tA : dy(); }
  const float* coef() const { return ws + w.acc; }
  const uint8_t* arg(int l) const { return reinterpret_cast<const uint8_t*>(ws + w.arg[l]); }
  int zero(void* p, size_t bytes, const char* who) const {
    if (bytes && hipMemsetAsync(p, 0, bytes, st) != hipSuccess) {
      set_error("%s: memset failed", who);
      return GCMI_ERR_LAUNCH;
    }
    return GCMI_OK;
  }
};

static void make_blocks(Step& s) {
  const gcmi_model_desc* m = s.m;
  const int L = m->n_layers;
  auto grad = [&](int64_t off) { return s.d_grads ? s.d_grads + off : nullptr; };
  for (int l = 0; l <= L; ++l) {
    Block& b = s.blk[l];
    b.K = l == 0 ? m->n_feat_in : m->conv_width[l - 1];
    b.W = l == L ? m->dense_width : m->conv_width[l];
    b.w = s.d_params + (l == L ? m->off_dense_w : m->off_conv_w[l]);
    b.bias = l == L ? s.d_params + m->off_dense_b : s.ws + s.w.bsum[l];
    b.dw = grad(l == L ? m->off_dense_w : m->off_conv_w[l]);
    b.dbias = l == L ? grad(m->off_dense_b) : s.ws + s.w.dbsum[l];
    b.dbias_rows = l == L ? nullptr : grad(m->off_conv_b[l]);
    BnPoint& p = b.bn;
    p = BnPoint();
    p.n_feat = b.W;
    if (m->batch_norm) {
      p.gamma = s.d_params + m->off_bn_gamma[l]; p.beta = s.d_params + m->off_bn_beta[l];
      p.dgamma = grad(m->off_bn_gamma[l]); p.dbeta = grad(m->off_bn_beta[l]);
    }
    float* bnv = s.ws + s.w.bnv[l];
    p.mean = bnv; p.invstd = bnv + b.W; p.scale = bnv + 2 * b.W; p.shift = bnv + 3 * b.W;
    p.running_mean = s.io->d_bn_running_mean[l]; p.running_var = s.io->d_bn_running_var[l];
    p.batches_tracked = s.io->d_bn_batches_tracked[l];
    p.eps = m->bn_eps; p.momentum = m->bn_momentum;
  }
}

static void make_step(Step& s, const gcmi_model_desc* m, const gcmi_graph* g, const float* d_params, float* d_grads,
                      const gcmi_model_io* io, gcmi_stat_sync_fn sync, void* sync_ctx, bool exchange, void* stream) {
  s.m = m; s.g = g; s.io = io; s.d_params = d_params; s.d_grads = d_grads;
  s.st = (hipStream_t)stream;
  s.L = m->n_layers; s.storage = m->storage;
  s.N = g->n_atoms; s.B = g->n_mols; s.nN = (int32_t)s.N;
  s.w = carve(m, s.N, s.B, io->ld_features);
  s.ws = io->d_workspace;
  make_blocks(s);
  s.acc = reinterpret_cast<double*>(s.ws + s.w.acc);
  s.acc2 = reinterpret_cast<double*>(s.ws + s.w.acc2);
  s.lacc = reinterpret_cast<double*>(s.ws + s.w.lacc);
  s.sync_s = BnSync{sync, sync_ctx, reinterpret_cast<double*>(s.ws + s.w.xch)};
  s.sy = exchange ? &s.sync_s : nullptr;
  s.training = 0; s.stats = nullptr;
  s.d_labels = s.d_weights = nullptr; s.n_rows = 0; s.grad_lo = s.grad_hi = nullptr; s.loss_inv_count = 0.f;
  s.full = m->grad_mode == 1;
  s.sym = g->d_rev_pos != nullptr || g->n_edges == 0;
  s.one_piece = false;
  memset(&s.ub, 0, sizeof(s.ub));
}

template <typename TA, typename TO>
static SegProduct<TA, TO> seg_product(const Segs& sg, const TA* a, int64_t lda, int32_t k, const float* w,
                                      const int64_t* w_off, int32_t n_out, TO* out) {
  SegProduct<TA, TO> p;
  p.n_seg = sg.n;
  p.seg_begin = sg.begin;
  p.seg_end = sg.end;
  p.op[0] = {a, lda, k, w, w_off};
  p.n_out = n_out;
  p.out = out;
  p.ldo = n_out;
  return p;
}

template <typename TA, typename TO>
static SegProduct<TA, TO> conv_product(const Segs& sg, const TA* s, int64_t lds, const TA* x, int64_t ldx, const Block& b,
                                       TO* out) {
  SegProduct<TA, TO> p = seg_product(sg, s, lds, b.K, b.w, sg.w_rel, b.W, out);
  p.op[1] = {x, ldx, b.K, b.w, sg.w_self};
  p.bias = b.bias;
  p.bias_off = sg.b_off;
  p.act = 1;
  return p;
}


static int pack_biases(const Step& s) {
  BiasLayers bl;
  memset(&bl, 0, sizeof(bl));
  for (int l = 0; l < s.L; ++l) {
    bl.src[l] = s.d_params + s.m->off_conv_b[l];
    bl.dst[l] = s.ws + s.w.bsum[l];
    bl.width[l] = s.m->conv_width[l];
  }
  hipLaunchKernelGGL(bias_pack_kernel, dim3(4, s.L), dim3(256), 0, s.st, bl, s.m->max_deg);
  GCMI_CHECK_LAUNCH("bias_pack");
  return GCMI_OK;
}

static int unpack_bias_grads(const Step& s) {
  bool any = false;
  for (int l = 0; l < s.L; ++l) any = any || s.ub.src[l] != nullptr;
  if (!any) return GCMI_OK;
  hipLaunchKernelGGL(bias_unpack_kernel, dim3(4, s.L), dim3(256), 0, s.st, s.ub, s.m->max_deg);
  GCMI_CHECK_LAUNCH("bias_unpack");
  return GCMI_OK;
}


static int bn_forward(const Step& s, const Block& b, bool stats_fused, const float* rows, int64_t ld) {
  const BnPoint& p = b.bn;
  if (!s.training)
    return gcmi_bn_fold_eval(p.gamma, p.beta, p.running_mean, p.running_var, p.eps, p.n_feat, p.scale, p.shift, s.st);
  BnForward f;
  f.x = rows; f.ldx = ld; f.sums_ready = stats_fused; f.n_rows = s.N; f.acc = s.acc; f.sync = s.sy;
  f.acc_clean = true;
  return bn_train_forward(p, f, s.st);
}

static int bump_counters(const Step& s) {
  CounterPtrs c;
  c.n = s.L + 1;
  bool any = false;
  for (int i = 0; i <= kMaxL; ++i) {
    c.p[i] = i <= s.L ? s.io->d_bn_batches_tracked[i] : nullptr;
    any = any || c.p[i] != nullptr;
  }
  if (any) {
    hipLaunchKernelGGL(bump_counters_kernel, dim3(1), dim3(64), 0, s.st, c);
    GCMI_CHECK_LAUNCH("bump_counters");
  }
  return GCMI_OK;
}

static int begin_forward(Step& s, int32_t training) {
  s.training = training;
  s.stats = (s.bn() && training) ? s.acc : nullptr;
  if (training && s.bn() && s.N > 0)
    RUN(s.zero(s.ws + s.w.acc, sizeof(float) * (size_t)(s.w.z_end - s.w.acc), "model_forward"));
  return pack_biases(s);
}

static int head_forward(const Step& s) {
  const gcmi_model_desc* m = s.m;
  const int D = m->dense_width;
  const int TC = m->n_tasks * m->n_classes;
  const int32_t nB = (int32_t)s.B;
  const float* hw = s.d_params + m->off_head_w;
  const float* hb = s.d_params + m->off_head_b;
  if (s.w.himg >= 0 && s.B > 0) {
    int rc = head_prep(hw, TC, s.ws + s.w.himg, s.st);
    if (rc == GCMI_OK)
      rc = head_fwd_wide(s.io->d_fingerprint, 2 * D, s.B, 2 * D, hw, hb, TC, 0, s.io->d_logits, TC, s.st, s.ws + s.w.himg);
    if (rc != GCMI_ERR_UNSUPPORTED) return rc;
  }
  SegProduct<float> p = one_segment(&nB, s.io->d_fingerprint, 2 * D, 2 * D, hw, hb, TC, s.io->d_logits, TC);
  p.trans_w = 1;
  return seg_gemm(p, s.st);
}

static int forward_tail(const Step& s) {
  const gcmi_model_desc* m = s.m;
  const Ws& w = s.w;
  const Block& dn = s.blk[s.L];
  const int D = dn.W;
  const bool h = s.storage != 0;
  bool stats_fused = h;
  if (s.N > 0 && h) {
    TimedScope ts(GCMI_K_SEG_GEMM, s.st);
    SegProduct<bf16_t> p = one_segment(&s.nN, (const bf16_t*)s.H(w.pool[s.L - 1]), (int64_t)dn.K, dn.K, dn.w, dn.bias, D,
                                       s.H(w.dense), D);
    p.trans_w = 1;
    p.act = 1;
    const int rc = fwd_h_gemm(p, s.stats, s.ws + w.wimg, s.st);
    if (rc == GCMI_ERR_UNSUPPORTED) set_error("bf16 activation storage: the dense layer has no bf16 product kernel");
    RUN(rc);
  } else if (s.N > 0) {
    SegProduct<float> p = one_segment(&s.nN, s.HF(w.pool[s.L - 1]), (int64_t)dn.K, dn.K, dn.w, dn.bias, D, s.ws + w.dense, D);
    p.trans_w = 1;
    p.act = 1;
    RUN(seg_gemm_stats(p, s.stats, &stats_fused, s.st));
  }
  const bool bn = s.bn() && s.N > 0;
  if (bn || s.sy) RUN(bn_forward(s, dn, stats_fused, h ? nullptr : s.ws + w.dense, h ? 0 : D));
  RUN(readout_fwd_impl(s.g, s.HF(w.dense), D, D, bn ? dn.bn.scale : nullptr, bn ? dn.bn.shift : nullptr, 1,
                       s.io->d_fingerprint, 2 * D, reinterpret_cast<int32_t*>(s.ws + w.arg_r),
                       (s.training && s.bn()) ? s.ws + w.rsum : nullptr, s.st, h ? 1 : 0));
  RUN(head_forward(s));
  if (m->mode == 0 && s.io->d_probs) RUN(gcmi_softmax(s.io->d_logits, s.B * m->n_tasks, m->n_classes, s.io->d_probs, s.st));
  if (s.training && s.bn() && s.N == 0 && !s.sy) RUN(bump_counters(s));
  return GCMI_OK;
}

// ... 93 lines not shown
static int model_forward_h(Step& s, int32_t training) {
  RUN(require_h(s.m, s.g, s.io, false));
  const gcmi_graph* g = s.g;
  const Ws& w = s.w;
  RUN(begin_forward(s, training));
  const bf16_t* xin = nullptr;
  int64_t ldin = 0;
  for (int l = 0; l < s.L; ++l) {
    const Block& b = s.blk[l];
    const Segs sg = make_segs(g, b.K, b.W);
    if (s.N > 0) {
      {
        TimedScope ts(GCMI_K_GATHER_SUM, s.st);
        if (l == 0) {
          RUN(win_gather_sum_fh(g, s.io->d_atom_features, s.io->ld_features, (int)w.ngather[0], s.H(w.S[0]), s.H(w.xb),
                                w.ldS[0], s.st));
          xin = s.H(w.xb);
          ldin = w.ldS[0];
        } else {
          RUN(win_gather_sum_h(g, xin, ldin, b.K, s.H(w.S[l]), w.ldS[l], s.st));
        }
      }
      {
        TimedScope ts(GCMI_K_SEG_GEMM, s.st);
        const int rc = fwd_h_gemm(conv_product(sg, (const bf16_t*)s.H(w.S[l]), w.ldS[l], xin, ldin, b, s.H(w.gc[l])),
                                  s.stats, s.ws + w.wimg, s.st);
        if (rc == GCMI_ERR_UNSUPPORTED) set_error("bf16 activation storage: GraphConv %d has no bf16 product kernel", l);
        RUN(rc);
      }
      RUN(bn_forward(s, b, true, nullptr, 0));
      {
        TimedScope ts(GCMI_K_GATHER_MAX, s.st);
        RUN(win_gather_max_h(g, s.H(w.gc[l]), b.W, b.W, b.bn.scale, b.bn.shift, s.H(w.pool[l]), b.W,
                             training ? reinterpret_cast<uint8_t*>(s.ws + w.arg[l]) : nullptr, s.st));
      }
    } else if (s.sy) {
      RUN(bn_forward(s, b, true, nullptr, 0));
    }
    xin = s.H(w.pool[l]);
    ldin = b.W;
  }
  return forward_tail(s);
}


static int begin_backward(Step& s) {
  const gcmi_model_desc* m = s.m;
  s.loss_inv_count = 1.f / (float)(s.n_rows * m->n_tasks);
  s.one_piece = s.storage == 0 && noted_one_piece(s.ws);
  const int64_t lo = s.full ? 0 : (s.bn() ? m->off_bn_gamma[s.L - 1] : m->off_dense_w);
  const int64_t hi = m->n_params;
  if (s.grad_lo) *s.grad_lo = lo;
  if (s.grad_hi) *s.grad_hi = hi;
  RUN(s.zero(s.d_grads + lo, sizeof(float) * (size_t)(hi - lo), "model_loss_backward"));
  RUN(s.zero(s.ws + s.w.dlogits, sizeof(float) * (size_t)(s.w.z_end - s.w.dlogits), "model_loss_backward"));
  const int D = m->dense_width;
  s.rg = ReadoutGrad{s.g->d_membership, s.ws + s.w.dfp, 2 * (int64_t)D, reinterpret_cast<const int32_t*>(s.ws + s.w.arg_r)};
  s.rg.rawsum = s.ws + s.w.rsum; s.rg.runs = s.g->d_mol_runs; s.rg.n_mols = s.g->n_mols; s.rg.n_deg = s.g->max_deg + 1;
  return GCMI_OK;
}

static int empty_backward_syncs(const Step& s) {
  for (int l = s.L; l >= 0; --l) {
    RUN(bn_bwd_sync_empty(s.blk[l].W, *s.sy, s.st));
    if (!s.full && l < s.L) break;
  }
  return GCMI_OK;
}

static int check_sync_buffers(const gcmi_model_desc* m, const gcmi_graph* g, const gcmi_model_io* io) {
  if (!aligned16(io->d_workspace)) {
    set_error("synchronised BatchNorm: the workspace must be 16-byte aligned");
    return GCMI_ERR_UNSUPPORTED;
  }
  const int64_t ldmax = std::max<int64_t>(2 * (int64_t)m->dense_width, std::max<int64_t>(io->ld_features, kOnePieceLd));
  if (fused_bwd_enabled() && (int64_t)g->n_atoms * ldmax >= (int64_t)1 << 30) {
    set_error("synchronised BatchNorm: %lld atoms per rank are beyond the one-pass block kernels (rows x row length "
              "below 2^30); use smaller shards", (long long)g->n_atoms);
    return GCMI_ERR_UNSUPPORTED;
  }
  return GCMI_OK;
}

static int refuse_second_sync(const char* what) {
  set_error("synchronised BatchNorm: %s refused its buffers, and the separate pass would exchange this BatchNorm's sums "
            "twice (16-byte aligned workspace and feature rows needed)", what);
  return GCMI_ERR_UNSUPPORTED;
}


static BnBackward bn_backward(const Step& s, const float* x, int64_t ldx, const BnSync* sy) {
  BnBackward q;
  q.x = x; q.ldx = ldx; q.n_rows = s.N; q.acc = s.acc; q.acc_clean = true; q.sync = sy;
  return q;
}

static int head_backward_fused(const Step& s, double* sums, bool* done, bool* with_sums) {
  const gcmi_model_desc* m = s.m;
  const BnPoint& dense_bn = s.blk[s.L].bn;
  HeadBackward h;
  h.kind = m->mode == 0 ? 0 : 1; h.logits = s.io->d_logits; h.labels = s.d_labels; h.weights = s.d_weights;
  h.n_rows = s.n_rows; h.n_tasks = m->n_tasks; h.n_classes = m->n_classes;
  h.fp = s.io->d_fingerprint; h.ldfp = 2 * dense_bn.n_feat;
  h.w = s.d_params + m->off_head_w; h.dw = s.d_grads + m->off_head_w; h.db = s.d_grads + m->off_head_b;
  h.rg = &s.rg; h.g2 = s.ws + s.w.dfp; h.loss_acc = s.lacc; h.dense_bn = &dense_bn; h.sums = sums;
  h.dl_scratch = s.ws + s.w.dlogits; h.img = s.w.himg >= 0 ? s.ws + s.w.himg : nullptr;
  *done = *with_sums = false;
  const int rc = head_bwd_fused(h, s.st);
// ... 228 lines not shown
  if (!s.sym) RUN(gcmi_scatter_add(g, dS, K, K, dX, K, s.st));
  return GCMI_OK;
}

static int model_loss_backward_f(Step& s) {
  RUN(begin_backward(s));
  const bool dense_one_pass = dense_block_one_pass(s.m, s.N);
  bool head_sums = false;
  RUN(head_backward(s, dense_one_pass, &head_sums));
  if (s.N == 0) return s.sy ? empty_backward_syncs(s) : GCMI_OK;
  bool have_psums = false;
  bool dy_ready = false;
  RUN(dense_block_backward(s, dense_one_pass, head_sums, &have_psums));
  for (int l = s.L - 1; l >= 0; --l) {
    if (!s.full && !s.bn()) break;
    const Block& b = s.blk[l];
    const Segs sg = make_segs(s.g, b.K, b.W);
    const BlockIn in = block_in(s, l);
    const BlockRoute r = block_route(s, l, in, have_psums);
    RUN(pool_bn_backward(s, l, r, dy_ready));
    have_psums = dy_ready = false;
    if (!s.full) break;
    bool one_pass_done = false;
    if (r.one_pass) RUN(conv_one_pass(s, l, sg, in, r, &one_pass_done));
    if (!one_pass_done && r.one_piece) {
      set_error("model_loss_backward: the forward left the first block's operands as bf16 rows, and the one-pass "
                "backward that reads them is not available now (GCMI_OPT_FUSED_BWD / GCMI_OPT_GEMM_EXACT changed?)");
      return GCMI_ERR_UNSUPPORTED;
    }
    if (!one_pass_done) RUN(conv_separate(s, l, sg, in));
    else if (l > 0) RUN(neighbour_part(s, l, r, &dy_ready));
    have_psums = one_pass_done && l > 0 && s.sym && s.bn();
    s.ub.src[l] = b.dbias; s.ub.dst[l] = b.dbias_rows; s.ub.width[l] = b.W;
  }
  return unpack_bias_grads(s);
}

static int model_loss_backward_h(Step& s) {
  RUN(require_h(s.m, s.g, s.io, true));
  return model_loss_backward_f(s);
}

}

using namespace gcmi;

extern "C" {

int gcmi_count_not_small_int(const float* d_x, int64_t ld, int64_t n_rows, int32_t n_cols, int32_t max_deg,
                             int64_t* d_count, void* stream) {
  GCMI_CHECK_ARG(d_count != nullptr && n_rows >= 0 && n_cols >= 0 && ld >= n_cols, "count_not_small_int: bad shape");
  GCMI_CHECK_ARG(n_rows * (int64_t)n_cols == 0 || d_x != nullptr, "count_not_small_int: NULL matrix");
  hipStream_t st = (hipStream_t)stream;
  if (hipMemsetAsync(d_count, 0, sizeof(int64_t), st) != hipSuccess) {
    set_error("count_not_small_int: memset failed");
    return GCMI_ERR_LAUNCH;
  }
  if (n_rows * (int64_t)n_cols == 0) return GCMI_OK;
  const float limit = (float)(256 / std::max(1, max_deg));
  hipLaunchKernelGGL(small_int_count_kernel, dim3(grid_for(n_rows * (int64_t)n_cols, 256)), dim3(256), 0, st, d_x, ld, n_rows,
                     n_cols, limit, reinterpret_cast<unsigned long long*>(d_count));
  GCMI_CHECK_LAUNCH("count_not_small_int");
  return GCMI_OK;
}

int64_t gcmi_model_workspace_floats(const gcmi_model_desc* m, int64_t n_atoms, int64_t n_mols) {
  if (check_desc(m) != GCMI_OK || n_atoms < 0 || n_mols < 0) return -1;
  return carve(m, n_atoms, n_mols, up4(m->n_feat_in)).total;
}


int gcmi_model_forward(const gcmi_model_desc* m, const gcmi_graph* g, const float* d_params,
                       const gcmi_model_io* io, int32_t training, void* stream) {
  return gcmi_model_forward_dp(m, g, d_params, io, training, nullptr, nullptr, stream);
}

int gcmi_model_forward_dp(const gcmi_model_desc* m, const gcmi_graph* g, const float* d_params,
                          const gcmi_model_io* io, int32_t training, gcmi_stat_sync_fn sync, void* sync_ctx,
                          void* stream) {
  RUN(check_desc(m));
  GCMI_CHECK_ARG(sync == nullptr || m->batch_norm, "model_forward_dp: a statistics exchange for a model without BatchNorm");
  RUN(check_graph(g, true));
  GCMI_CHECK_ARG(io && d_params && io->d_workspace && io->d_logits && io->d_fingerprint,
                 "model_forward: NULL buffer");
  GCMI_CHECK_ARG(g->max_deg == m->max_deg, "graph max_deg %d != model max_deg %d", g->max_deg, m->max_deg);
  GCMI_CHECK_ARG(g->n_mols > 1, "graph_gather requires batches larger than 1");
  GCMI_CHECK_ARG(g->n_atoms == 0 || io->d_atom_features, "model_forward: NULL atom features");
  GCMI_CHECK_ARG(io->ld_features >= m->n_feat_in, "ld_features < n_feat_in");
  if (sync && training) RUN(check_sync_buffers(m, g, io));
  Step s;
  make_step(s, m, g, d_params, nullptr, io, sync, sync_ctx, sync && training, stream);
  return m->storage >= 1 ? model_forward_h(s, training) : model_forward_f(s, training);
}

int gcmi_model_loss_backward(const gcmi_model_desc* m, const gcmi_graph* g, const float* d_params,
                             float* d_grads, const gcmi_model_io* io, const float* d_labels,
                             const float* d_weights, int64_t n_rows, int64_t* grad_lo,
                             int64_t* grad_hi, void* stream) {
  return gcmi_model_loss_backward_dp(m, g, d_params, d_grads, io, d_labels, d_weights, n_rows, grad_lo, grad_hi, nullptr,
                                     nullptr, stream);
}

int gcmi_model_loss_backward_dp(const gcmi_model_desc* m, const gcmi_graph* g, const float* d_params,
                                float* d_grads, const gcmi_model_io* io, const float* d_labels,
                                const float* d_weights, int64_t n_rows, int64_t* grad_lo, int64_t* grad_hi,
                                gcmi_stat_sync_fn sync, void* sync_ctx, void* stream) {
  RUN(check_desc(m));
// ... 17 lines not shown
```

### deepchem_amd/csrc/readout.hip

```cpp
#include <limits.h>
#include <math.h>

#include <atomic>

#include "common.h"
#include "split_bf16.h"

namespace gcmi {

constexpr int kRBlock = 256;

__global__ void __launch_bounds__(kRBlock)
mol_runs_kernel(DegTable t, int n_atoms, int n_mols, const int32_t* __restrict__ membership,
                int32_t* __restrict__ runs, int32_t* __restrict__ flag) {
  const int n_deg = t.max_deg + 1;
  for (int i = blockIdx.x * kRBlock + threadIdx.x; i < n_atoms; i += gridDim.x * kRBlock) {
    const int d = degree_of_row(t, i);
    int lo = 0, hi = 0;
#pragma unroll
    for (int k = 0; k <= GCMI_MAX_DEG; ++k) {
      if (k == d) {
        lo = t.deg_start[k];
        hi = t.deg_start[k + 1];
      }
// ... 216 lines not shown
      }
    }
#pragma unroll
    for (int q = 0; q < V; ++q) {
      float s1 = gs[q], m1 = gm[q];
      if (act == 1) {
        s1 *= (1.f - os[q] * os[q]);
        m1 *= (1.f - om[q] * om[q]);
      }
      g[q] = s1 + ((am[q] == i) ? m1 : 0.f);
    }
    if constexpr (V == 4) {
      *reinterpret_cast<float4*>(dx + (int64_t)i * lddx + c) = make_float4(g[0], g[1], g[2], g[3]);
    } else {
      dx[(int64_t)i * lddx + c] = g[0];
    }
  }
}

__global__ void readout_grad_prep_kernel(float* __restrict__ g, int64_t ldg, const float* __restrict__ out,
                                         int64_t ldo, int64_t n_mols, int n2) {
  const int64_t total = n_mols * n2;
  for (int64_t e = (int64_t)blockIdx.x * blockDim.x + threadIdx.x; e < total; e += (int64_t)gridDim.x * blockDim.x) {
    const int64_t b = e / n2;
    const int c = (int)(e - b * n2);
    const float o = out[b * ldo + c];
    g[b * ldg + c] *= (1.f - o * o);
  }
}

int readout_grad_prep(float* d_g, int64_t ldg, const float* d_out, int64_t ldo, int64_t n_mols, int n_feat,
                      hipStream_t st) {
  if (n_mols == 0) return GCMI_OK;
  hipLaunchKernelGGL(readout_grad_prep_kernel, dim3(grid_for(n_mols * 2 * n_feat, 256)), dim3(256), 0, st, d_g, ldg,
                     d_out, ldo, n_mols, 2 * n_feat);
  GCMI_CHECK_LAUNCH("readout_grad_prep");
  return GCMI_OK;
}

}

using namespace gcmi;

extern "C" {

int gcmi_build_mol_runs(const gcmi_graph* g, int32_t* d_mol_runs, int32_t* d_flag, void* stream) {
  int rc = check_graph(g, false);
  if (rc) return rc;
  GCMI_CHECK_ARG(d_mol_runs != nullptr || g->n_mols == 0, "build_mol_runs: NULL output");
  GCMI_CHECK_ARG(g->n_atoms == 0 || g->d_membership != nullptr, "build_mol_runs: d_membership is NULL");
  hipStream_t st = (hipStream_t)stream;
  const size_t bytes = (size_t)g->n_mols * (g->max_deg + 1) * 2 * sizeof(int32_t);
  if (bytes) {
    if (hipMemsetAsync(d_mol_runs, 0, bytes, st) != hipSuccess) {
      set_error("build_mol_runs: memset failed");
      return GCMI_ERR_LAUNCH;
    }
  }
  if (d_flag && hipMemsetAsync(d_flag, 0, sizeof(int32_t), st) != hipSuccess) {
    set_error("build_mol_runs: memset failed");
    return GCMI_ERR_LAUNCH;
  }
  if (g->n_atoms == 0) return GCMI_OK;
  DegTable t = make_deg_table(g);
  hipLaunchKernelGGL(mol_runs_kernel, dim3(grid_for(g->n_atoms, kRBlock)), dim3(kRBlock), 0, st, t,
                     g->n_atoms, g->n_mols, g->d_membership, d_mol_runs, d_flag);
  GCMI_CHECK_LAUNCH("build_mol_runs");
  return GCMI_OK;
}

int gcmi_readout_fwd(const gcmi_graph* g, const float* d_x, int64_t ldx, int32_t n_feat,
                     const float* d_scale, const float* d_shift, int32_t act, float* d_out,
                     int64_t ldo, int32_t* d_arg, void* stream) {
  return gcmi::readout_fwd_impl(g, d_x, ldx, n_feat, d_scale, d_shift, act, d_out, ldo, d_arg, nullptr, stream);
}

}

namespace gcmi {
static std::atomic<int> g_readout_pre{getenv("GCMI_READOUT_PRE") && atoi(getenv("GCMI_READOUT_PRE")) == 0 ? 0 : 1};
void set_readout_pipelined(int on) { g_readout_pre.store(on ? 1 : 0, std::memory_order_relaxed); }
int get_readout_pipelined() { return g_readout_pre.load(std::memory_order_relaxed); }

int readout_fwd_impl(const gcmi_graph* g, const float* d_x, int64_t ldx, int32_t n_feat, const float* d_scale,
                     const float* d_shift, int32_t act, float* d_out, int64_t ldo, int32_t* d_arg, float* d_rawsum,
                     void* stream, int32_t x_bf16) {
  int rc = check_graph(g, false);
  if (rc) return rc;
  GCMI_CHECK_ARG(n_feat > 0 && ldx >= n_feat && ldo >= 2 * (int64_t)n_feat, "readout: bad n_feat/ld");
  GCMI_CHECK_ARG(g->n_mols == 0 || (d_out && g->d_mol_runs), "readout: NULL output or mol runs");
  GCMI_CHECK_ARG(g->n_atoms == 0 || d_x, "readout: NULL input");
  GCMI_CHECK_ARG((d_scale == nullptr) == (d_shift == nullptr), "readout: scale/shift must come together");
  GCMI_CHECK_ARG(act == 0 || act == 1, "readout: act must be 0 or 1");
  if (g->n_mols == 0) return GCMI_OK;
  hipStream_t st = (hipStream_t)stream;
  const int V = x_bf16 ? ((reinterpret_cast<uintptr_t>(d_x) & 7u) == 0 && ldx % 4 == 0 && n_feat % 4 == 0 ? 4 : 1)
                       : vec_width(d_x, ldx, n_feat);
  if (x_bf16 && V != 4) {
    set_error("readout (bf16 rows): rows must be 8-byte addressable");
    return GCMI_ERR_UNSUPPORTED;
  }
  const int lpr = n_feat / V;
  const int gl = lpr < kRBlock ? lpr : kRBlock;
  const int tb = kRBlock;
  const int mpb = tb / gl;
  const int blocks = (g->n_mols + mpb - 1) / mpb;
  const bool bn = d_scale != nullptr;
  const int n_deg = g->max_deg + 1;
  const int vec_out = (n_feat % 4 == 0 && ldo % 4 == 0 && aligned16(d_out) && (d_arg == nullptr || aligned16(d_arg)) &&
                       (d_rawsum == nullptr || aligned16(d_rawsum)))
                          ? 1
                          : 0;
// ... 105 lines not shown
```

### deepchem_amd/ops.py

```python
import ctypes
from typing import Optional

import numpy as np
import torch

from deepchem_amd import _lib
from deepchem_amd.graph import BatchGraph, _stream

_vp = ctypes.c_void_p


def _ptr(t: Optional[torch.Tensor]):
    return None if t is None else _vp(t.data_ptr())


def _mat(t: torch.Tensor, name: str, rows: Optional[int] = None, cols: Optional[int] = None,
         dtype=torch.float32):
    if not torch.is_tensor(t) or not t.is_cuda:
        raise _lib.GcmiError("%s must be a CUDA tensor: the hot path has no CPU implementation" % name)
    if t.dtype != dtype:
        raise TypeError("%s must be %s, got %s" % (name, dtype, t.dtype))
    if t.dim() != 2 or (t.numel() > 0 and t.shape[1] > 1 and t.stride(1) != 1):
        raise ValueError("%s must be 2-D with unit column stride (shape %s, strides %s)" %
                         (name, tuple(t.shape), t.stride()))
# ... 42 lines not shown
    _mat(ds, "ds", rows=g.n_atoms)
    _mat(dx, "dx", rows=g.n_atoms, cols=ds.shape[1])
    _lib.call("gcmi_scatter_add", g.ref, _ptr(ds), _ld(ds), ds.shape[1], _ptr(dx), _ld(dx), _stream())
    return dx


def _arg_rows(arg, n_atoms: int, n_feat: int):
    if arg.dtype != torch.uint8 or tuple(arg.shape) != (n_atoms, n_feat) or not arg.is_contiguous() or not arg.is_cuda:
        raise ValueError("bad arg tensor")
    return arg


def _out_rows(out, like: torch.Tensor, n_atoms: int, n_feat: int, name: str = "out"):
    if out is None:
        return torch.empty((n_atoms, n_feat), dtype=like.dtype, device=like.device)
    return _mat(out, name, rows=n_atoms, cols=n_feat, dtype=like.dtype)


def gather_max(g: BatchGraph, x: torch.Tensor, scale=None, shift=None, want_arg: bool = True, out=None, arg=None):
    _mat(x, "x", rows=g.n_atoms)
    F_ = x.shape[1]
    _vec(scale, "scale", F_)
    _vec(shift, "shift", F_)
    out = _out_rows(out, x, g.n_atoms, F_)
    if arg is not None:
        _arg_rows(arg, g.n_atoms, F_)
    elif want_arg:
        arg = torch.empty((g.n_atoms, F_), dtype=torch.uint8, device=x.device)
    _lib.call("gcmi_gather_max_fwd", g.ref, _ptr(x), _ld(x), F_, _ptr(scale), _ptr(shift), _ptr(out),
              _ld(out), _ptr(arg), _stream())
    return out, arg


def gather_max_sum(g: BatchGraph, y: torch.Tensor, scale=None, shift=None, want_arg: bool = True, pool=None, arg=None,
                   s=None):
    _mat(y, "y", rows=g.n_atoms)
    F_ = y.shape[1]
    _vec(scale, "scale", F_)
    _vec(shift, "shift", F_)
    pool = _out_rows(pool, y, g.n_atoms, F_, "pool")
    if arg is not None:
        _arg_rows(arg, g.n_atoms, F_)
    elif want_arg:
        arg = torch.empty((g.n_atoms, F_), dtype=torch.uint8, device=y.device)
    s = _out_rows(s, y, g.n_atoms, F_, "s")
    _lib.call("gcmi_gather_max_sum_fwd", g.ref, _ptr(y), _ld(y), F_, _ptr(scale), _ptr(shift), _ptr(pool),
              _ld(pool), _ptr(arg), _ptr(s), _ld(s), _stream())
    return pool, arg, s


def max_sum_launches() -> int:
    v = ctypes.c_int32(0)
    _lib.call("gcmi_get_option", _lib.GCMI_OPT_MAX_SUM_LAUNCHES, ctypes.byref(v))
    return v.value


def gather_max_bwd(g: BatchGraph, dout: torch.Tensor, arg: torch.Tensor, out=None) -> torch.Tensor:
    _mat(dout, "dout", rows=g.n_atoms)
    F_ = dout.shape[1]
    if arg.dtype != torch.uint8 or tuple(arg.shape) != (g.n_atoms, F_) or not arg.is_contiguous():
        raise ValueError("bad arg tensor")
    if g.ensure_rev_pos():
        dx = _out_rows(out, dout, g.n_atoms, F_, "out")
    else:
        if out is not None:
            raise ValueError("out needs a graph with reverse slots")
        dx = torch.zeros((g.n_atoms, F_), dtype=torch.float32, device=dout.device)
    _lib.call("gcmi_gather_max_bwd", g.ref, _ptr(dout), _ld(dout), F_, _ptr(arg), _ptr(dx), _ld(dx),
              _stream())
    return dx


_BF16 = torch.bfloat16


def win_sum_h(g: BatchGraph, x: torch.Tensor, out: Optional[torch.Tensor] = None, accumulate: bool = False):
    _mat(x, "x", rows=g.n_atoms, dtype=_BF16)
    F_ = x.shape[1]
    if out is None and accumulate:
        raise ValueError("accumulate needs an output")
    out = _out_rows(out, x, g.n_atoms, F_)
    _lib.call("gcmi_win_sum_h", g.ref, _ptr(x), _ld(x), F_, _ptr(out), _ld(out), 1 if accumulate else 0, _stream())
    return out


def win_sum_fh(g: BatchGraph, x: torch.Tensor, ldo: int, s=None, xcopy=None):
    _mat(x, "x", rows=g.n_atoms)
    F_ = x.shape[1]
    outs = []
    for t, name in ((s, "s"), (xcopy, "xcopy")):
        if t is None:
            t = torch.empty((g.n_atoms, ldo), dtype=_BF16, device=x.device)
        _mat(t, name, rows=g.n_atoms, cols=ldo, dtype=_BF16)
        if _ld(t) != ldo:
            raise ValueError("%s: row stride %d, expected %d" % (name, _ld(t), ldo))
        outs.append(t)
    _lib.call("gcmi_win_sum_fh", g.ref, _ptr(x), _ld(x), F_, _ptr(outs[0]), _ptr(outs[1]), int(ldo), _stream())
    return outs[0], outs[1]


def win_max_h(g: BatchGraph, x: torch.Tensor, scale=None, shift=None, want_arg: bool = True, out=None, arg=None):
    _mat(x, "x", rows=g.n_atoms, dtype=_BF16)
    F_ = x.shape[1]
    _vec(scale, "scale", F_)
    _vec(shift, "shift", F_)
    out = _out_rows(out, x, g.n_atoms, F_)
# ... 1222 lines not shown
```

### include/gcmi.h

```cpp
#ifndef GCMI_H
#define GCMI_H

#include <stddef.h>
#include <stdint.h>

#ifdef __cplusplus
extern "C" {
#endif

#define GCMI_VERSION 100
#define GCMI_MAX_DEG 10

typedef enum gcmi_status {
  GCMI_OK = 0,
  GCMI_ERR_ARG = -1,
  GCMI_ERR_LAUNCH = -2,
  GCMI_ERR_UNSUPPORTED = -3
} gcmi_status;

#define GCMI_WIN_META_INTS 24
#define GCMI_WIN_SLOT_BITS 12
#define GCMI_WIN_MAX_SLOTS 4095

typedef struct gcmi_graph {
  int32_t n_atoms;
  int32_t n_edges;
  int32_t n_mols;
  int32_t max_deg;
  int32_t deg_start[GCMI_MAX_DEG + 2];
  int32_t edge_start[GCMI_MAX_DEG + 2];
  const int32_t* d_col_idx;
  const int32_t* d_membership;
  const int32_t* d_mol_runs;
  const uint8_t* d_rev_pos;
  int32_t n_win;
  int32_t n_win_big;
  int32_t win_alloc;
  int32_t win_ecap;
  int32_t win_alloc_big;
  int32_t win_ecap_big;
  int32_t win_reserved[2];
  const int32_t* d_win_meta;
  const uint16_t* d_win_edges;
} gcmi_graph;

int gcmi_version(void);
enum {
  GCMI_OPT_GEMM_EXACT = 1,
  GCMI_OPT_FUSED_BN_STATS = 2,
  GCMI_OPT_FUSED_BWD = 3,
  GCMI_OPT_FUSED_BWD_LAUNCHES = 4,
  GCMI_OPT_READOUT_PIPELINED = 5,
  GCMI_OPT_ONE_PIECE_LAUNCHES = 6,
  GCMI_OPT_MAX_SUM_LAUNCHES = 7
};
int gcmi_set_option(int32_t option, int32_t value);
int gcmi_get_option(int32_t option, int32_t* value);
const char* gcmi_last_error(void);

int gcmi_collate_sizes(const int64_t* atom_ptr, const int64_t* adj_ptr, const int64_t* sel,
                       int64_t n_sel, int64_t* out_n_atoms, int64_t* out_n_edges);
int gcmi_collate(const float* atom_features, int64_t n_feat, const int64_t* atom_ptr,
                 const int64_t* adj_ptr, const int32_t* adj_idx, const int64_t* sel,
                 int64_t n_sel, int32_t max_deg, float* out_features, int64_t out_ld,
                 int64_t cap_atoms, int32_t* out_membership, int32_t* out_col_idx,
                 int64_t cap_edges, int32_t* out_mol_runs, gcmi_graph* graph);
int gcmi_collate_plans(const float* atom_features, int64_t n_feat, const int64_t* atom_ptr,
                       const int64_t* adj_ptr, const int32_t* adj_idx, const int64_t* sel,
                       int64_t n_sel, int32_t max_deg, float* out_features, int64_t out_ld,
                       int64_t cap_atoms, int32_t* out_membership, int32_t* out_col_idx,
                       int64_t cap_edges, int32_t* out_mol_runs, uint8_t* out_rev_pos,
                       int32_t* out_symmetric, int32_t win_cap, int32_t* out_win_meta,
                       uint16_t* out_win_edges, gcmi_graph* graph);
int gcmi_collate_plans_p(const float* atom_features, int64_t n_feat, const int64_t* atom_ptr,
                         const int64_t* adj_ptr, const int32_t* adj_idx, const int64_t* sel,
                         int64_t n_sel, int32_t max_deg, float* out_features, int64_t out_ld,
                         int64_t cap_atoms, int32_t* out_membership, int32_t* out_col_idx,
                         int64_t cap_edges, int32_t* out_mol_runs, uint8_t* out_rev_pos,
                         int32_t* out_symmetric, int32_t win_cap, int32_t* out_win_meta,
                         uint16_t* out_win_edges, gcmi_graph* graph, int32_t atom_codes, int32_t* out_small_int);

#define GCMI_COLLATE_WIN_DESC_INTS 36
int gcmi_molset_tables(const int64_t* atom_ptr, const int64_t* adj_ptr, const int32_t* adj_idx, int64_t n_mols,
                       int32_t max_deg, int32_t* out_mol_hist, int32_t* out_rank, uint8_t* out_rev,
                       int32_t* out_symmetric, int32_t n_threads);
int64_t gcmi_collate_plan_words(int64_t n_sel);
int gcmi_collate_plan(const int32_t* mol_hist, const int64_t* atom_ptr, const int64_t* sel, int64_t n_sel,
                      int32_t max_deg, int32_t win_cap, int32_t* staging, int64_t staging_words,
                      int64_t* out_offsets, gcmi_graph* graph);
int gcmi_collate_rows(const void* d_features, int64_t n_feat, const int64_t* d_adj_ptr, const int32_t* d_adj_idx,
                      const int32_t* d_rank, const uint8_t* d_rev, const int32_t* d_staging,
                      const int64_t* offsets, const gcmi_graph* plan, float* d_out_features, int64_t out_ld,
                      int32_t* d_membership, int32_t* d_col_idx, int32_t* d_mol_runs, uint8_t* d_rev_pos,
                      uint16_t* d_win_edges, int64_t* d_src_atom, void* stream);
int gcmi_collate_rows_host(const void* features, int64_t n_feat, const int64_t* adj_ptr, const int32_t* adj_idx,
                           const int32_t* rank, const uint8_t* rev, const int32_t* staging, const int64_t* offsets,
                           const gcmi_graph* plan, float* out_features, int64_t out_ld, int32_t* membership,
                           int32_t* col_idx, int32_t* mol_runs, uint8_t* rev_pos, uint16_t* win_edges);

int gcmi_build_mol_runs(const gcmi_graph* g, int32_t* d_mol_runs, int32_t* d_flag, void* stream);
int gcmi_build_rev_pos(const gcmi_graph* g, uint8_t* d_rev_pos, int32_t* d_flag, void* stream);

int gcmi_gather_sum_fwd(const gcmi_graph* g, const float* d_x, int64_t ldx, int32_t n_feat,
                        float* d_s, int64_t lds, int32_t accumulate ,
                        void* stream);
int gcmi_scatter_add(const gcmi_graph* g, const float* d_ds, int64_t ldds, int32_t n_feat,
                     float* d_dx, int64_t lddx, void* stream);
// ... 379 lines not shown
```

Measured before the change: 22.63 million molecules/s.

## Cut per-step launches: fold memsets into kernels, handle oversized windows in-kernel

Adds a native launch counter and cuts launches per training step. The workspace clear is folded into the bias-pack kernel, and the two backward memsets become one zeroing kernel. The window gather kernels now process oversized windows in a single launch with two phases (first, publish stores with fences, restage, second), replacing the extra fallback launches. This targets launch and queue overhead, at the cost of device fences and restaging inside the big-window path.

```diff
diff --git a/deepchem_amd/_lib.py b/deepchem_amd/_lib.py
--- a/deepchem_amd/_lib.py
+++ b/deepchem_amd/_lib.py
@@ -20,6 +20,7 @@
 GCMI_OPT_READOUT_PIPELINED = 5
 GCMI_OPT_ONE_PIECE_LAUNCHES = 6
 GCMI_OPT_MAX_SUM_LAUNCHES = 7
+GCMI_OPT_LAUNCHES = 8
 GCMI_METRIC_ROC_AUC, GCMI_METRIC_PRC_AUC = 0, 1
 GCMI_METRIC_MOMENTS, GCMI_METRIC_ACCURACY = 0, 1
 GCMI_METRIC_MOMENT_DOUBLES = 12
diff --git a/deepchem_amd/csrc/bn.hip b/deepchem_amd/csrc/bn.hip
--- a/deepchem_amd/csrc/bn.hip
+++ b/deepchem_amd/csrc/bn.hip
@@ -398,7 +398,7 @@
                            double* sums, bool acc_clean, hipStream_t st, const ReadoutGrad* rgp = nullptr,
                            const float* only_if_gamma = nullptr, const float* only_if_beta = nullptr, int x_bf16 = 0) {
   if (!acc_clean &&
-      hipMemsetAsync(sums, 0, sizeof(double) * 2 * n_feat * (1 + kReplicas), st) != hipSuccess) {
+      memset_async(sums, 0, sizeof(double) * 2 * n_feat * (1 + kReplicas), st) != hipSuccess) {
     set_error("bn: memset failed");
     return GCMI_ERR_LAUNCH;
   }
@@ -459,7 +459,7 @@
 
 static int bn_sync_exchange(const BnSync& sy, int64_t n_rows, int32_t n_feat, hipStream_t st) {
   const int64_t n = 2 * (int64_t)n_feat + 1;
-  if (n_rows == 0 && hipMemsetAsync(sy.buf, 0, sizeof(double) * (size_t)n, st) != hipSuccess) {
+  if (n_rows == 0 && memset_async(sy.buf, 0, sizeof(double) * (size_t)n, st) != hipSuccess) {
     set_error("bn sync: memset failed");
     return GCMI_ERR_LAUNCH;
   }
@@ -783,7 +783,7 @@
   int rc = GCMI_OK;
   if (rgp && rgp->rawsum && rgp->runs && rgp->n_mols > 0) {
     if (!b.acc_clean &&
-        hipMemsetAsync(b.acc, 0, sizeof(double) * 2 * n_feat * (1 + kReplicas), st) != hipSuccess) {
+        memset_async(b.acc, 0, sizeof(double) * 2 * n_feat * (1 + kReplicas), st) != hipSuccess) {
       set_error("bn: memset failed");
       return GCMI_ERR_LAUNCH;
     }
diff --git a/deepchem_amd/csrc/bwd_fused.hip b/deepchem_amd/csrc/bwd_fused.hip
--- a/deepchem_amd/csrc/bwd_fused.hip
+++ b/deepchem_amd/csrc/bwd_fused.hip
@@ -595,7 +595,7 @@
   FusedArgs aa = a;
   if (diag_on) {
     if (!d_diag && hipMalloc(&d_diag, 10 * sizeof(unsigned long long)) != hipSuccess) d_diag = nullptr;
-    if (d_diag) (void)hipMemsetAsync(d_diag, 0, 10 * sizeof(unsigned long long), sm);
+    if (d_diag) (void)memset_async(d_diag, 0, 10 * sizeof(unsigned long long), sm);
     aa.diag = d_diag;
   }
   hipLaunchKernelGGL(kern, dim3(grid), dim3(DGRAD ? 512 : 256), shmem, sm, st, n_tiles, aa, next_sweep_direction());
diff --git a/deepchem_amd/csrc/collate.cpp b/deepchem_amd/csrc/collate.cpp
--- a/deepchem_amd/csrc/collate.cpp
+++ b/deepchem_amd/csrc/collate.cpp
@@ -762,7 +762,7 @@
                                 d_out_features, out_ld, d_membership, d_col_idx, d_mol_runs, d_rev_pos, d_win_edges);
   if (rc != GCMI_OK) return rc;
   if (A.want_win && offsets[7] > 0)
-    if (hipMemsetAsync(d_win_edges, 0, (size_t)offsets[7] * sizeof(uint16_t), stream) != hipSuccess) {
+    if (::gcmi::memset_async(d_win_edges, 0, (size_t)offsets[7] * sizeof(uint16_t), stream) != hipSuccess) {
       ::gcmi::set_error("collate_rows: hipMemsetAsync failed");
       return GCMI_ERR_LAUNCH;
     }
diff --git a/deepchem_amd/csrc/common.h b/deepchem_amd/csrc/common.h
--- a/deepchem_amd/csrc/common.h
+++ b/deepchem_amd/csrc/common.h
@@ -28,8 +28,16 @@
     }                                      \
   } while (0)
 
+void count_launch();
+int native_launches();
+inline hipError_t memset_async(void* p, int value, size_t bytes, hipStream_t st) {
+  count_launch();
+  return hipMemsetAsync(p, value, bytes, st);
+}
+
 #define GCMI_CHECK_LAUNCH(what)                                                        \
   do {                                                                                 \
+    ::gcmi::count_launch();                                                            \
     hipError_t e__ = hipGetLastError();                                                \
     if (e__ != hipSuccess) {                                                           \
       ::gcmi::set_error("%s: %s", what, hipGetErrorString(e__));                       \
diff --git a/deepchem_amd/csrc/core.cpp b/deepchem_amd/csrc/core.cpp
--- a/deepchem_amd/csrc/core.cpp
+++ b/deepchem_amd/csrc/core.cpp
@@ -13,6 +13,10 @@
 
 static std::atomic<unsigned> g_sweep_counter{0};
 int next_sweep_direction() { return (int)(g_sweep_counter.fetch_add(1, std::memory_order_relaxed) & 1u); }
+
+static std::atomic<int> g_launches{0};
+void count_launch() { g_launches.fetch_add(1, std::memory_order_relaxed); }
+int native_launches() { return g_launches.load(std::memory_order_relaxed); }
 
 int raise_lds_limit(LdsLimit& a, const void* kern, size_t lds_bytes, int threads, size_t shmem) {
   int dev = -1;
diff --git a/deepchem_amd/csrc/gather.hip b/deepchem_amd/csrc/gather.hip
--- a/deepchem_amd/csrc/gather.hip
+++ b/deepchem_amd/csrc/gather.hip
@@ -447,7 +447,7 @@
   if (rc) return rc;
   GCMI_CHECK_ARG(d_flag != nullptr, "build_rev_pos: d_flag is NULL");
   hipStream_t st = (hipStream_t)stream;
-  if (hipMemsetAsync(d_flag, 0, sizeof(int32_t), st) != hipSuccess) {
+  if (memset_async(d_flag, 0, sizeof(int32_t), st) != hipSuccess) {
     set_error("build_rev_pos: memset failed");
     return GCMI_ERR_LAUNCH;
   }
diff --git a/deepchem_amd/csrc/gather_lds.hip b/deepchem_amd/csrc/gather_lds.hip
--- a/deepchem_amd/csrc/gather_lds.hip
+++ b/deepchem_amd/csrc/gather_lds.hip
@@ -458,7 +458,7 @@
 template <class T>
 struct SumAccMaxBwdBody {
   using P = Piece<T>;
-  const T* __restrict__ dxs;
+  const T* dxs;
   int64_t lddxs;
   T* __restrict__ dy;
   int64_t lddy;
@@ -480,12 +480,37 @@
       t2[e] = P::narrow(acc);
     }
     __syncthreads();
+    pool_bwd_rows<WT, LPR>(t2, w, L, m);
+  }
+  template <int WT, int LPR>
+  __device__ __forceinline__ void pool_bwd_rows(const typename P::Raw* dx, const WinBuf<P>& w, const Layout& L,
+                                                const WinMeta& m) const {
     for (int e = threadIdx.x; e < w.n16; e += WT) {
       const PieceAt at = piece_at<LPR>(m, L.maxd, e);
       typename P::Vals acc;
-      pool_bwd<P, LPR>(t2, w.aux, w.ent + at.eloc, at.d, e, at.c, acc);
+      pool_bwd<P, LPR>(dx, w.aux, w.ent + at.eloc, at.d, e, at.c, acc);
       store_piece(dy + (int64_t)at.row * lddy + at.c * P::kEPP, acc);
     }
+  }
+  __device__ __forceinline__ const char* mid_src() const { return reinterpret_cast<const char*>(dxs); }
+  __device__ __forceinline__ int64_t mid_ld_bytes() const { return lddxs * (int64_t)sizeof(T); }
+  template <int WT, int LPR>
+  __device__ __forceinline__ void first(const char* buf, const Layout& L, const WinMeta& m, const float*) const {
+    const WinBuf<P> w = open_buf<P, LPR>(buf, L, m);
+    for (int e = threadIdx.x; e < w.n16; e += WT) {
+      const PieceAt at = piece_at<LPR>(m, L.maxd, e);
+      T* dst = const_cast<T*>(dxs) + (int64_t)at.row * lddxs + at.c * P::kEPP;
+      const typename P::Raw old = load_piece(dst);
+      typename P::Vals acc;
+      neigh_sum<P, LPR>(w.tile, w.ent + at.eloc, at.d, at.c, acc);
+      add_piece<P>(acc, old);
+      store_piece(dst, acc);
+    }
+  }
+  template <int WT, int LPR>
+  __device__ __forceinline__ void second(const char* buf, const Layout& L, const WinMeta& m) const {
+    const WinBuf<P> w = open_buf<P, LPR>(buf, L, m);
+    pool_bwd_rows<WT, LPR>(w.tile, w, L, m);
   }
 };
 
@@ -521,12 +546,28 @@
       t2[e] = P::narrow(best);
     }
     __syncthreads();
+    sum_rows<WT, LPR>(t2, w, L, m);
+  }
+  template <int WT, int LPR>
+  __device__ __forceinline__ void sum_rows(const typename P::Raw* pooled, const WinBuf<P>& w, const Layout& L,
+                                           const WinMeta& m) const {
     for (int e = threadIdx.x; e < w.n16; e += WT) {
       const PieceAt at = piece_at<LPR>(m, L.maxd, e);
       typename P::Vals acc;
-      neigh_sum<P, LPR>(t2, w.ent + at.eloc, at.d, at.c, acc);
+      neigh_sum<P, LPR>(pooled, w.ent + at.eloc, at.d, at.c, acc);
       store_piece(s + (int64_t)at.row * lds + at.c * P::kEPP, acc);
     }
+  }
+  __device__ __forceinline__ const char* mid_src() const { return reinterpret_cast<const char*>(pool.out); }
+  __device__ __forceinline__ int64_t mid_ld_bytes() const { return pool.ldo * (int64_t)sizeof(T); }
+  template <int WT, int LPR>
+  __device__ __forceinline__ void first(const char* buf, const Layout& L, const WinMeta& m, const float* sh_lds) const {
+    pool.template run<WT, LPR>(buf, L, m, sh_lds);
+  }
+  template <int WT, int LPR>
+  __device__ __forceinline__ void second(const char* buf, const Layout& L, const WinMeta& m) const {
+    const WinBuf<P> w = open_buf<P, LPR>(buf, L, m);
+    sum_rows<WT, LPR>(w.tile, w, L, m);
   }
 };
 
@@ -534,6 +575,16 @@
 struct MaxSumOp : MaxSumBody<float, BN> {
   static constexpr int kThreads = WT;
 };
+
+
+__device__ __forceinline__ void publish_own_stores() {
+  wait_dma();
+  __builtin_amdgcn_fence(__ATOMIC_RELEASE, "agent");
+  wait_dma();
+  __syncthreads();
+  __builtin_amdgcn_fence(__ATOMIC_ACQUIRE, "agent");
+  wait_dma();
+}
 
 template <int WT, int LPR, bool AUX, class Op>
 __global__ void __launch_bounds__(WT)
@@ -564,7 +615,16 @@
       stage<WT, LPR, AUX, kEPP>(smem, Lbig, m, x, ldx, aux, edges);
       wait_dma();
       __syncthreads();
-      compute(smem, Lbig, m, smem + 2 * L.buf_bytes());
+      if constexpr (kXT || kScratch) {
+        op.template first<WT, LPR>(smem, Lbig, m, op_lds);
+        publish_own_stores();
+        stage<WT, LPR, AUX, kEPP>(smem, Lbig, m, op.mid_src(), op.mid_ld_bytes(), aux, edges);
+        wait_dma();
+        __syncthreads();
+        op.template second<WT, LPR>(smem, Lbig, m);
+      } else {
+        compute(smem, Lbig, m, nullptr);
+      }
       __syncthreads();
     }
     return;
@@ -656,7 +716,7 @@
 
 template <int LPR, bool AUX, class Op>
 static int launch_lpr(const gcmi_graph* g, const WinPlan& p, const char* x, int64_t ldx, const uint8_t* aux,
-                      const Op& op, hipStream_t st, const char* what, int which) {
+                      const Op& op, hipStream_t st, const char* what) {
   constexpr int WT = Op::kThreads;
   auto kern = win_kernel<WT, LPR, AUX, Op>;
   static LdsLimit lim;
@@ -667,21 +727,20 @@
   const int n_norm = g->n_win - g->n_win_big;
   size_t shmem = p.shmem;
   if constexpr (Op::kThird != Third::none) {
-    if (which != 1) {
-      set_error("%s: oversized windows are not handled by the two-stage form", what);
-      return GCMI_ERR_UNSUPPORTED;
-    }
     shmem += (size_t)p.L.tile_bytes * third_tiles(Op::kThird);
     if (shmem > (size_t)kLdsPerCU) return GCMI_ERR_UNSUPPORTED;
   }
   const int by_lds = (int)((size_t)kLdsPerCU / shmem);
   const int by_threads = 2048 / WT;
   const int per_cu = std::max(1, std::min(8, std::min(by_lds, by_threads)));
-  const int g_norm = which == 2 ? 0 : std::min(n_norm, 256 * per_cu);
-  const int g_big = which == 1 ? 0 : std::min(g->n_win_big, 64);
+  const int g_norm = std::min(n_norm, 256 * per_cu);
+  const int g_big = std::min(g->n_win_big, 64);
   if (g_norm + g_big == 0) return GCMI_OK;
+  int turns = 1;
+  if constexpr (Op::kThird != Third::none)
+    turns = (g_norm > 0 ? (Op::kThird == Third::scratch ? 2 : 1) : 0) + (g_big > 0 ? 2 : 0);
   const int rev = next_sweep_direction();
-  if constexpr (Op::kThird == Third::scratch) (void)next_sweep_direction();
+  for (int i = 1; i < turns; ++i) (void)next_sweep_direction();
   hipLaunchKernelGGL(kern, dim3(g_norm + g_big), dim3(WT), shmem, st, g->d_win_meta, g->d_win_edges, n_norm,
                      g->n_win, g_norm, p.L, p.Lbig, x, ldx, aux, op, rev);
   GCMI_CHECK_LAUNCH(what);
@@ -690,35 +749,29 @@
 
 template <bool AUX, class T, class Op>
 static int launch(const gcmi_graph* g, int n_feat, const T* x, int64_t ldx, const uint8_t* aux, const Op& op,
-                  hipStream_t st, const char* what, int which = 0) {
+                  hipStream_t st, const char* what) {
   using P = Piece<T>;
   constexpr bool kH = P::kEPP == 8;
   const WinPlan p = make_plan(g, n_feat * (int)sizeof(T) / 4, AUX ? P::kEPP : 0);
   const char* xb = reinterpret_cast<const char*>(x);
   const int64_t ldb = ldx * (int64_t)sizeof(T);
   switch (n_feat / P::kEPP) {
-    case 8: if constexpr (kH) return launch_lpr<8, AUX, Op>(g, p, xb, ldb, aux, op, st, what, which); break;
-    case 10: if constexpr (kH) return launch_lpr<10, AUX, Op>(g, p, xb, ldb, aux, op, st, what, which); break;
-    case 16: return launch_lpr<16, AUX, Op>(g, p, xb, ldb, aux, op, st, what, which);
-    case 19: if constexpr (!kH) return launch_lpr<19, AUX, Op>(g, p, xb, ldb, aux, op, st, what, which); break;
-    case 32: if constexpr (!kH) return launch_lpr<32, AUX, Op>(g, p, xb, ldb, aux, op, st, what, which); break;
+    case 8: if constexpr (kH) return launch_lpr<8, AUX, Op>(g, p, xb, ldb, aux, op, st, what); break;
+    case 10: if constexpr (kH) return launch_lpr<10, AUX, Op>(g, p, xb, ldb, aux, op, st, what); break;
+    case 16: return launch_lpr<16, AUX, Op>(g, p, xb, ldb, aux, op, st, what);
+    case 19: if constexpr (!kH) return launch_lpr<19, AUX, Op>(g, p, xb, ldb, aux, op, st, what); break;
+    case 32: if constexpr (!kH) return launch_lpr<32, AUX, Op>(g, p, xb, ldb, aux, op, st, what); break;
     default: break;
   }
   set_error(kH ? "%s: no bf16 window kernel for %d features" : "%s: no window kernel for %d features", what, n_feat);
   return GCMI_ERR_UNSUPPORTED;
 }
 
-template <class TwoStage, class SumAcc, class Bwd, class T>
+template <class TwoStage, class T>
 static int sumacc_max_bwd(const gcmi_graph* g, const T* d_ds, int64_t ldds, int n_feat, T* d_dxs, int64_t lddxs,
-                          const uint8_t* d_arg, T* d_dy, int64_t lddy, hipStream_t st, const char* const (&what)[3]) {
+                          const uint8_t* d_arg, T* d_dy, int64_t lddy, hipStream_t st, const char* what) {
   TwoStage op{{d_dxs, lddxs, d_dy, lddy}};
-  int rc = launch<true>(g, n_feat, d_ds, ldds, d_arg, op, st, what[0], 1);
-  if (rc || g->n_win_big == 0) return rc;
-  SumAcc acc{{d_dxs, lddxs}};
-  rc = launch<false>(g, n_feat, d_ds, ldds, nullptr, acc, st, what[1], 2);
-  if (rc) return rc;
-  Bwd mb{{d_dy, lddy, nullptr, nullptr}};
-  return launch<true>(g, n_feat, d_dxs, lddxs, d_arg, mb, st, what[2], 2);
+  return launch<true>(g, n_feat, d_ds, ldds, d_arg, op, st, what);
 }
 
 bool win_has_width(int n_feat) { return n_feat == 64 || n_feat == 76 || n_feat == 128; }
@@ -766,10 +819,8 @@
 
 int win_gather_sumacc_max_bwd(const gcmi_graph* g, const float* d_ds, int64_t ldds, int n_feat, float* d_dxs,
                               int64_t lddxs, const uint8_t* d_arg, float* d_dy, int64_t lddy, hipStream_t st) {
-  return sumacc_max_bwd<SumAccMaxBwdOp, SumOp<true>, MaxBwdOp>(
-      g, d_ds, ldds, n_feat, d_dxs, lddxs, d_arg, d_dy, lddy, st,
-      {"win_gather_sumacc_max_bwd", "win_gather_sum (accumulate, oversized windows)",
-       "win_gather_max_bwd (oversized windows)"});
+  return sumacc_max_bwd<SumAccMaxBwdOp>(g, d_ds, ldds, n_feat, d_dxs, lddxs, d_arg, d_dy, lddy, st,
+                                        "win_gather_sumacc_max_bwd");
 }
 
 bool win_max_sum_usable(const gcmi_graph* g, int n_feat) {
@@ -788,11 +839,11 @@
   const int64_t ldb = ldy * (int64_t)sizeof(float);
   if (n_feat == 128) {
     MaxSumOp<BN, 1024> op{{pool, d_s, lds}};
-    return launch_lpr<32, false>(g, p, yb, ldb, nullptr, op, st, "win_gather_max_sum", 1);
+    return launch_lpr<32, false>(g, p, yb, ldb, nullptr, op, st, "win_gather_max_sum");
   }
   if (n_feat == 64) {
     MaxSumOp<BN, 512> op{{pool, d_s, lds}};
-    return launch_lpr<16, false>(g, p, yb, ldb, nullptr, op, st, "win_gather_max_sum", 1);
+    return launch_lpr<16, false>(g, p, yb, ldb, nullptr, op, st, "win_gather_max_sum");
   }
   set_error("win_gather_max_sum: no window kernel for %d features", n_feat);
   return GCMI_ERR_UNSUPPORTED;
@@ -803,19 +854,8 @@
                        hipStream_t st) {
   int rc = d_scale ? max_sum<true>(g, d_y, ldy, n_feat, {d_scale, d_shift, d_pool, ldp, d_arg}, d_s, lds, st)
                    : max_sum<false>(g, d_y, ldy, n_feat, {nullptr, nullptr, d_pool, ldp, d_arg}, d_s, lds, st);
-  if (rc) return rc;
-  if (g->n_win > g->n_win_big) g_max_sum_launches.fetch_add(1, std::memory_order_relaxed);
-  if (g->n_win_big == 0) return rc;
-  if (d_scale) {
-    MaxOp<true> mx{{d_scale, d_shift, d_pool, ldp, d_arg}};
-    rc = launch<false>(g, n_feat, d_y, ldy, nullptr, mx, st, "win_gather_max (oversized windows)", 2);
-  } else {
-    MaxOp<false> mx{{nullptr, nullptr, d_pool, ldp, d_arg}};
-    rc = launch<false>(g, n_feat, d_y, ldy, nullptr, mx, st, "win_gather_max (oversized windows)", 2);
-  }
-  if (rc) return rc;
-  SumOp<false> sm{{d_s, lds}};
-  return launch<false>(g, n_feat, d_pool, ldp, nullptr, sm, st, "win_gather_sum (oversized windows)", 2);
+  if (rc == GCMI_OK && g->n_win > g->n_win_big) g_max_sum_launches.fetch_add(1, std::memory_order_relaxed);
+  return rc;
 }
 
 bool win_usable_h(const gcmi_graph* g, int n_feat) {
@@ -875,10 +915,8 @@
 
 int win_gather_sumacc_max_bwd_h(const gcmi_graph* g, const bf16_t* d_ds, int64_t ldds, int n_feat, bf16_t* d_dxs,
                                 int64_t lddxs, const uint8_t* d_arg, bf16_t* d_dy, int64_t lddy, hipStream_t st) {
-  return sumacc_max_bwd<SumAccMaxBwdOpH, SumAccOpH, MaxBwdOpH>(
-      g, d_ds, ldds, n_feat, d_dxs, lddxs, d_arg, d_dy, lddy, st,
-      {"win_gather_sumacc_max_bwd (bf16)", "win_gather_sum (bf16, accumulate, oversized windows)",
-       "win_gather_max_bwd (bf16, oversized windows)"});
-}
-
-}
+  return sumacc_max_bwd<SumAccMaxBwdOpH>(g, d_ds, ldds, n_feat, d_dxs, lddxs, d_arg, d_dy, lddy, st,
+                                         "win_gather_sumacc_max_bwd (bf16)");
+}
+
+}
diff --git a/deepchem_amd/csrc/gemm.hip b/deepchem_amd/csrc/gemm.hip
--- a/deepchem_amd/csrc/gemm.hip
+++ b/deepchem_amd/csrc/gemm.hip
@@ -567,7 +567,8 @@
 int gcmi_get_option(int32_t option, int32_t* value) {
   GCMI_CHECK_ARG((option == GCMI_OPT_GEMM_EXACT || option == GCMI_OPT_FUSED_BN_STATS || option == GCMI_OPT_FUSED_BWD ||
                   option == GCMI_OPT_FUSED_BWD_LAUNCHES || option == GCMI_OPT_READOUT_PIPELINED ||
-                  option == GCMI_OPT_ONE_PIECE_LAUNCHES || option == GCMI_OPT_MAX_SUM_LAUNCHES) && value,
+                  option == GCMI_OPT_ONE_PIECE_LAUNCHES || option == GCMI_OPT_MAX_SUM_LAUNCHES ||
+                  option == GCMI_OPT_LAUNCHES) && value,
                  "get_option: unknown option %d", option);
   if (option == GCMI_OPT_GEMM_EXACT) *value = g_gemm_exact.load(std::memory_order_relaxed);
   else if (option == GCMI_OPT_FUSED_BN_STATS) *value = g_fused_bn_stats.load(std::memory_order_relaxed);
@@ -575,6 +576,7 @@
   else if (option == GCMI_OPT_READOUT_PIPELINED) *value = get_readout_pipelined();
   else if (option == GCMI_OPT_ONE_PIECE_LAUNCHES) *value = one_piece_launches();
   else if (option == GCMI_OPT_MAX_SUM_LAUNCHES) *value = max_sum_launches();
+  else if (option == GCMI_OPT_LAUNCHES) *value = native_launches();
   else *value = fused_bwd_launches();
   return GCMI_OK;
 }
diff --git a/deepchem_amd/csrc/loss.hip b/deepchem_amd/csrc/loss.hip
--- a/deepchem_amd/csrc/loss.hip
+++ b/deepchem_amd/csrc/loss.hip
@@ -109,7 +109,7 @@
   GCMI_CHECK_ARG(n_rows > 0 && n_tasks > 0 && (kind == 1 || n_classes > 0), "loss: bad shape");
   GCMI_CHECK_ARG(d_logits && d_labels && d_loss && d_acc, "loss: NULL buffer");
   hipStream_t st = (hipStream_t)stream;
-  if (!acc_clean && hipMemsetAsync(d_acc, 0, sizeof(double), st) != hipSuccess) {
+  if (!acc_clean && memset_async(d_acc, 0, sizeof(double), st) != hipSuccess) {
     set_error("loss: memset failed");
     return GCMI_ERR_LAUNCH;
   }
diff --git a/deepchem_amd/csrc/metrics.hip b/deepchem_amd/csrc/metrics.hip
--- a/deepchem_amd/csrc/metrics.hip
+++ b/deepchem_amd/csrc/metrics.hip
@@ -362,7 +362,7 @@
   GCMI_CHECK_ARG(aligned16(d_workspace), "metric_rank: workspace must be 16-byte aligned");
   hipStream_t st = (hipStream_t)stream;
   RankWorkspace ws = carve(d_workspace, n, n_tasks);
-  if (hipMemsetAsync(d_status, 0, sizeof(int32_t) * n_tasks, st) != hipSuccess) {
+  if (memset_async(d_status, 0, sizeof(int32_t) * n_tasks, st) != hipSuccess) {
     set_error("metric_rank: memset failed");
     return GCMI_ERR_LAUNCH;
   }
@@ -405,7 +405,7 @@
   GCMI_CHECK_ARG(row_stride >= 0 && elem_stride >= 0, "metric_moments: negative stride");
   GCMI_CHECK_ARG(d_pred && d_labels && d_out, "metric_moments: NULL buffer");
   hipStream_t st = (hipStream_t)stream;
-  if (hipMemsetAsync(d_out, 0, sizeof(double) * GCMI_METRIC_MOMENT_DOUBLES * n_tasks, st) != hipSuccess) {
+  if (memset_async(d_out, 0, sizeof(double) * GCMI_METRIC_MOMENT_DOUBLES * n_tasks, st) != hipSuccess) {
     set_error("metric_moments: memset failed");
     return GCMI_ERR_LAUNCH;
   }
diff --git a/deepchem_amd/csrc/model.hip b/deepchem_amd/csrc/model.hip
--- a/deepchem_amd/csrc/model.hip
+++ b/deepchem_amd/csrc/model.hip
@@ -14,7 +14,19 @@
   int width[kMaxL];
 };
 
-__global__ void bias_pack_kernel(BiasLayers bl, int max_deg) {
+__device__ __forceinline__ void zero_floats(float* __restrict__ p, int64_t n, int64_t tid, int64_t nt) {
+  int64_t head = (int64_t)((16u - (unsigned)(reinterpret_cast<uintptr_t>(p) & 15u)) & 15u) / 4;
+  if (head > n) head = n;
+  const int64_t n4 = (n - head) / 4;
+  float4* __restrict__ q = reinterpret_cast<float4*>(p + head);
+  for (int64_t i = tid; i < head; i += nt) p[i] = 0.f;
+  for (int64_t i = tid; i < n4; i += nt) q[i] = make_float4(0.f, 0.f, 0.f, 0.f);
+  for (int64_t i = head + 4 * n4 + tid; i < n; i += nt) p[i] = 0.f;
+}
+
+__global__ void step_prep_kernel(BiasLayers bl, int max_deg, float* __restrict__ zero, int64_t n_zero) {
+  const int64_t nt = (int64_t)gridDim.x * gridDim.y * blockDim.x;
+  zero_floats(zero, n_zero, ((int64_t)blockIdx.y * gridDim.x + blockIdx.x) * blockDim.x + threadIdx.x, nt);
   const int l = blockIdx.y;
   const float* __restrict__ b_list = pick_n(bl.src, l);
   float* __restrict__ bsum = pick_n(bl.dst, l);
@@ -26,6 +38,13 @@
     bsum[i] = d == 0 ? b_list[(2 * max_deg) * width + c]
                      : b_list[(2 * (d - 1)) * width + c] + b_list[(2 * (d - 1) + 1) * width + c];
   }
+}
+
+__global__ void zero_pair_kernel(float* __restrict__ a, int64_t na, float* __restrict__ b, int64_t nb) {
+  const int64_t nt = (int64_t)gridDim.x * blockDim.x;
+  const int64_t tid = (int64_t)blockIdx.x * blockDim.x + threadIdx.x;
+  zero_floats(a, na, tid, nt);
+  zero_floats(b, nb, tid, nt);
 }
 
 __global__ void bias_unpack_kernel(BiasLayers bl, int max_deg) {
@@ -253,7 +272,7 @@
   const float* coef() const { return ws + w.acc; }
   const uint8_t* arg(int l) const { return reinterpret_cast<const uint8_t*>(ws + w.arg[l]); }
   int zero(void* p, size_t bytes, const char* who) const {
-    if (bytes && hipMemsetAsync(p, 0, bytes, st) != hipSuccess) {
+    if (bytes && memset_async(p, 0, bytes, st) != hipSuccess) {
       set_error("%s: memset failed", who);
       return GCMI_ERR_LAUNCH;
     }
@@ -337,7 +356,7 @@
 }
 
 
-static int pack_biases(const Step& s) {
+static int pack_biases(const Step& s, float* zero, int64_t n_zero) {
   BiasLayers bl;
   memset(&bl, 0, sizeof(bl));
   for (int l = 0; l < s.L; ++l) {
@@ -345,8 +364,8 @@
     bl.dst[l] = s.ws + s.w.bsum[l];
     bl.width[l] = s.m->conv_width[l];
   }
-  hipLaunchKernelGGL(bias_pack_kernel, dim3(4, s.L), dim3(256), 0, s.st, bl, s.m->max_deg);
-  GCMI_CHECK_LAUNCH("bias_pack");
+  hipLaunchKernelGGL(step_prep_kernel, dim3(4, s.L), dim3(256), 0, s.st, bl, s.m->max_deg, zero, n_zero);
+  GCMI_CHECK_LAUNCH("step_prep");
   return GCMI_OK;
 }
 
@@ -388,9 +407,8 @@
 static int begin_forward(Step& s, int32_t training) {
   s.training = training;
   s.stats = (s.bn() && training) ? s.acc : nullptr;
-  if (training && s.bn() && s.N > 0)
-    RUN(s.zero(s.ws + s.w.acc, sizeof(float) * (size_t)(s.w.z_end - s.w.acc), "model_forward"));
-  return pack_biases(s);
+  const bool clear = training && s.bn() && s.N > 0;
+  return pack_biases(s, s.ws + s.w.acc, clear ? s.w.z_end - s.w.acc : 0);
 }
 
 static int head_forward(const Step& s) {
@@ -590,8 +608,11 @@
   const int64_t hi = m->n_params;
   if (s.grad_lo) *s.grad_lo = lo;
   if (s.grad_hi) *s.grad_hi = hi;
-  RUN(s.zero(s.d_grads + lo, sizeof(float) * (size_t)(hi - lo), "model_loss_backward"));
-  RUN(s.zero(s.ws + s.w.dlogits, sizeof(float) * (size_t)(s.w.z_end - s.w.dlogits), "model_loss_backward"));
+  const int64_t n_ws = s.w.z_end - s.w.dlogits;
+  const int64_t blocks = std::min<int64_t>(1024, std::max<int64_t>(1, (hi - lo + n_ws) / (256 * 16)));
+  hipLaunchKernelGGL(zero_pair_kernel, dim3((unsigned)blocks), dim3(256), 0, s.st, s.d_grads + lo, hi - lo,
+                     s.ws + s.w.dlogits, n_ws);
+  GCMI_CHECK_LAUNCH("model_loss_backward: zero");
   const int D = m->dense_width;
   s.rg = ReadoutGrad{s.g->d_membership, s.ws + s.w.dfp, 2 * (int64_t)D, reinterpret_cast<const int32_t*>(s.ws + s.w.arg_r)};
   s.rg.rawsum = s.ws + s.w.rsum; s.rg.runs = s.g->d_mol_runs; s.rg.n_mols = s.g->n_mols; s.rg.n_deg = s.g->max_deg + 1;
@@ -926,7 +947,7 @@
   GCMI_CHECK_ARG(d_count != nullptr && n_rows >= 0 && n_cols >= 0 && ld >= n_cols, "count_not_small_int: bad shape");
   GCMI_CHECK_ARG(n_rows * (int64_t)n_cols == 0 || d_x != nullptr, "count_not_small_int: NULL matrix");
   hipStream_t st = (hipStream_t)stream;
-  if (hipMemsetAsync(d_count, 0, sizeof(int64_t), st) != hipSuccess) {
+  if (memset_async(d_count, 0, sizeof(int64_t), st) != hipSuccess) {
     set_error("count_not_small_int: memset failed");
     return GCMI_ERR_LAUNCH;
   }
diff --git a/deepchem_amd/csrc/readout.hip b/deepchem_amd/csrc/readout.hip
--- a/deepchem_amd/csrc/readout.hip
+++ b/deepchem_amd/csrc/readout.hip
@@ -292,12 +292,12 @@
   hipStream_t st = (hipStream_t)stream;
   const size_t bytes = (size_t)g->n_mols * (g->max_deg + 1) * 2 * sizeof(int32_t);
   if (bytes) {
-    if (hipMemsetAsync(d_mol_runs, 0, bytes, st) != hipSuccess) {
+    if (memset_async(d_mol_runs, 0, bytes, st) != hipSuccess) {
       set_error("build_mol_runs: memset failed");
       return GCMI_ERR_LAUNCH;
     }
   }
-  if (d_flag && hipMemsetAsync(d_flag, 0, sizeof(int32_t), st) != hipSuccess) {
+  if (d_flag && memset_async(d_flag, 0, sizeof(int32_t), st) != hipSuccess) {
     set_error("build_mol_runs: memset failed");
     return GCMI_ERR_LAUNCH;
   }
diff --git a/deepchem_amd/ops.py b/deepchem_amd/ops.py
--- a/deepchem_amd/ops.py
+++ b/deepchem_amd/ops.py
@@ -118,6 +118,12 @@
 def max_sum_launches() -> int:
     v = ctypes.c_int32(0)
     _lib.call("gcmi_get_option", _lib.GCMI_OPT_MAX_SUM_LAUNCHES, ctypes.byref(v))
+    return v.value
+
+
+def native_launches() -> int:
+    v = ctypes.c_int32(0)
+    _lib.call("gcmi_get_option", _lib.GCMI_OPT_LAUNCHES, ctypes.byref(v))
     return v.value
 
 
diff --git a/include/gcmi.h b/include/gcmi.h
--- a/include/gcmi.h
+++ b/include/gcmi.h
@@ -52,7 +52,8 @@
   GCMI_OPT_FUSED_BWD_LAUNCHES = 4,
   GCMI_OPT_READOUT_PIPELINED = 5,
   GCMI_OPT_ONE_PIECE_LAUNCHES = 6,
-  GCMI_OPT_MAX_SUM_LAUNCHES = 7
+  GCMI_OPT_MAX_SUM_LAUNCHES = 7,
+  GCMI_OPT_LAUNCHES = 8
 };
 int gcmi_set_option(int32_t option, int32_t value);
 int gcmi_get_option(int32_t option, int32_t* value);
```

Measured after the change: 22.74 million molecules/s (median of 3 runs). Within noise of the previous version (+0.5%).
